# smithzvk/gsl-scattered-interpolation

Measured on AMD Instinct MI355X. Metric: M interpolated points/sec (whole hot path: fill + solve + eval sweep per step), higher is better.
Workload: dtype f64; 1 GPU; C3: 3-D N=16384 Gaussian RBF (16k x 16k fp64 Cholesky), M=1M targets per GPU; config=C3, n_centres=16384, dim=3, targets_per_gpu=1000000, targets_total=1000000, parallelism=1 GPU

## Files before the change

gsl-scattered-interpolation_amd/csrc/hip/chol.hip:

```cpp
#include "common.h"
#include <math.h>
#include <stdlib.h>

#ifdef SINTERP_DIAG_PROF
__device__ unsigned long long g_diag_ts[80];
#define TSTAMP(i) do { if (threadIdx.x == 0) g_diag_ts[i] = __builtin_readcyclecounter(); } while (0)
extern "C" int gsl_sinterp_hip_debug_diag_ts(unsigned long long *out) { return (int)hipMemcpyFromSymbol(out, HIP_SYMBOL(g_diag_ts), sizeof(unsigned long long) * 80); }
#endif
#include "chol_potrf.h"

#define TRSV_MAXR 5


__global__ void __launch_bounds__(256)
chol_base_kernel(double *__restrict__ A, size_t lda, size_t n, size_t j0, int nb, int *__restrict__ info,
                 double *__restrict__ diag_store)
{
  __shared__ double sL[CB][CB + 1];
  __shared__ double sInv[CB];
  const int tid = threadIdx.x;

  const size_t row = j0 + nb + (size_t)blockIdx.x * blockDim.x + tid;
  double *p = A + row * lda + j0;
  double x[CB];
  const bool vecrow = nb == CB && ((((uintptr_t)p) & 15) == 0) && ((lda & 1) == 0);
  if (row < n) {
    if (vecrow) {
#pragma unroll
      for (int k = 0; k < CB; k += 2) { const double2 t = *reinterpret_cast<const double2 *>(p + k); x[k] = t.x; x[k + 1] = t.y; }
    } else {
#pragma unroll
      for (int k = 0; k < CB; k++) x[k] = k < nb ? p[k] : 0.0;
    }
  }

  if (tid < 64) {
    const int lane = tid;
    double a[CB];
#pragma unroll
    for (int k = 0; k < CB; k++) a[k] = (lane < nb && k <= lane && k < nb) ? A[(j0 + lane) * lda + j0 + k] : 0.0;
    bool bad = false;
#pragma unroll
    for (int j = 0; j < CB; j++) {
      double v = a[j];
#pragma unroll
      for (int k = 0; k < j; k++) v = fma(-a[k], lane_bcast(a[k], j), v);
      double d = lane_bcast(v, j);
      if (j < nb && !(d > 0.0)) {
        if (lane == 0 && blockIdx.x == 0) atomicCAS(info, 0, (int)(j0 + j + 1));
        bad = true;
        d = 1.0;
      }
      if (j >= nb) d = 1.0;
      double y = __builtin_amdgcn_rsq(d);
      y = y * fma(-0.5 * d * y, y, 1.5);
      y = y * fma(-0.5 * d * y, y, 1.5);
      double sd = d * y;
      sd = fma(fma(-sd, sd, d), 0.5 * y, sd);
      const double inv = fma(fma(-sd, y, 1.0), y, y);
      a[j] = (lane == j) ? sd : v * inv;
      if (lane == 0) sInv[j] = inv;
    }
    (void)bad;
    if (lane < CB) {
#pragma unroll
      for (int k = 0; k < CB; k++) sL[lane][k] = (k <= lane) ? a[k] : 0.0;
      if (blockIdx.x == 0) {
        double *dst = diag_store + (j0 / CB) * (CB * CB) + lane * CB;
#pragma unroll
        for (int k = 0; k < CB; k++) dst[k] = (k <= lane) ? a[k] : 0.0;
      }
    }
  }
  __syncthreads();

  if (row >= n) return;
#pragma unroll
  for (int j = 0; j < CB; j++) {
    double v = x[j];
#pragma unroll
    for (int k = 0; k < j; k++) v = fma(-x[k], sL[j][k], v);
    x[j] = v * sInv[j];
  }
  if (vecrow) {
#pragma unroll
    for (int k = 0; k < CB; k += 2) *reinterpret_cast<double2 *>(p + k) = make_double2(x[k], x[k + 1]);
  } else {
#pragma unroll
    for (int k = 0; k < CB; k++) if (k < nb) p[k] = x[k];
  }
}

__global__ void __launch_bounds__(256)
chol_diag_writeback_kernel(double *__restrict__ A, size_t lda, size_t n, const double *__restrict__ diag_store)
{
  const size_t j0 = (size_t)blockIdx.x * CB;
  for (int e = threadIdx.x; e < CB * CB; e += 256) {
    const int r = e / CB, k = e % CB;
    if (k <= r && j0 + r < n) A[(j0 + r) * lda + j0 + k] = diag_store[(size_t)blockIdx.x * (CB * CB) + e];
  }
}


__device__ __forceinline__ void diag128_forward(const double *S, const double *Dv, double *fs, double *tt, int tid, int nrhs)
{
  const int lane = tid & 63, wave = tid >> 6, r = lane & 31, half = lane >> 5;
  for (int q = wave; q < nrhs; q += 4) {
    double *y = fs + q * PB, *t = tt + q * CB;
#pragma unroll
    for (int i = 0; i < 4; i++) {
      double sum = 0.0;
#pragma unroll
      for (int kb = 0; kb < i; kb++) {
        const double *Lr = S + pblk(i, kb) + r * PQ + half * 16;
        const double *yk = y + kb * 32 + half * 16;
#pragma unroll
        for (int k = 0; k < 16; k += 2) {
          const double2 l2 = *reinterpret_cast<const double2 *>(Lr + k);
          sum = fma(l2.x, yk[k], sum);
          sum = fma(l2.y, yk[k + 1], sum);
        }
      }
      sum += __shfl_xor(sum, 32);
      if (half == 0) t[r] = y[i * 32 + r] - sum;
      __builtin_amdgcn_wave_barrier();
      const double *Wr = Dv + i * PBLK + (half * 16) * PQ + r;
      double acc = 0.0;
#pragma unroll
      for (int c = 0; c < 16; c++) acc = fma(Wr[c * PQ], t[half * 16 + c], acc);
      acc += __shfl_xor(acc, 32);
      if (half == 0) y[i * 32 + r] = acc;
      __builtin_amdgcn_wave_barrier();
    }
  }
}

__global__ void __launch_bounds__(256)
chol_diag128_kernel(double *__restrict__ A, size_t lda, size_t j0, int *__restrict__ info, double *__restrict__ diag_store,
                    double *__restrict__ Dinvg, double *__restrict__ fb, size_t ldf, int nrhs)
{
  extern __shared__ __attribute__((aligned(16))) double sm[];
  double *S = sm;
  double *Dv = S + 10 * PBLK;
  double *fs = Dv + 4 * PBLK;
  double *tt = fs + 5 * PB;
  const int tid = threadIdx.x;
  double *Ab = A + j0 * lda + j0;
  TSTAMP(0);

  {
    double v[40], fv[3];
    const int r8 = tid >> 5, k = tid & 31;
#pragma unroll
    for (int t = 0; t < 40; t++) {
      constexpr int BI[10] = {0, 1, 1, 2, 2, 2, 3, 3, 3, 3}, BJ[10] = {0, 0, 1, 0, 1, 2, 0, 1, 2, 3};
      const int b = t >> 2, r = (t & 3) * 8 + r8;
      v[t] = Ab[(size_t)(BI[b] * 32 + r) * lda + BJ[b] * 32 + k];
    }
#pragma unroll
    for (int t = 0; t < 3; t++) { const int e = t * 256 + tid; fv[t] = e < nrhs * PB ? fb[(size_t)(e >> 7) * ldf + j0 + (e & 127)] : 0.0; }
#pragma unroll
    for (int t = 0; t < 40; t++) S[(t >> 2) * PBLK + ((t & 3) * 8 + r8) * PQ + k] = v[t];
#pragma unroll
    for (int t = 0; t < 16; t++) { const int r = (t & 3) * 8 + r8; Dv[(t >> 2) * PBLK + r * PQ + k] = r == k ? 1.0 : 0.0; }
#pragma unroll
    for (int t = 0; t < 3; t++) { const int e = t * 256 + tid; if (e < nrhs * PB) fs[e] = fv[t]; }
  }
  __syncthreads();
  TSTAMP(1);

  potrf128_lds<4>(S, Dv, tid, info, j0);

  TSTAMP(18);
  if (nrhs > 0) {
    diag128_forward(S, Dv, fs, tt, tid, nrhs);
    __syncthreads();
  }
  {
    const int r8 = tid >> 5, k = tid & 31;
#pragma unroll
    for (int t = 0; t < 40; t++) {
      constexpr int BI[10] = {0, 1, 1, 2, 2, 2, 3, 3, 3, 3}, BJ[10] = {0, 0, 1, 0, 1, 2, 0, 1, 2, 3};
      const int b = t >> 2, r = (t & 3) * 8 + r8, bi = BI[b], bj = BJ[b];
      const double v = S[b * PBLK + r * PQ + k];
      if (bi != bj || k <= r) Ab[(size_t)(bi * 32 + r) * lda + bj * 32 + k] = v;
      if (bi == bj && diag_store) diag_store[(j0 / CB + bi) * (CB * CB) + r * CB + k] = (k <= r) ? v : 0.0;
    }
#pragma unroll
    for (int t = 0; t < 16; t++) {
      const int b = t >> 2, r = (t & 3) * 8 + r8;
      Dinvg[b * 1024 + r * 32 + k] = Dv[b * PBLK + k * PQ + r];
    }
#pragma unroll
    for (int t = 0; t < 3; t++) { const int e = t * 256 + tid; if (e < nrhs * PB) fb[(size_t)(e >> 7) * ldf + j0 + (e & 127)] = fs[e]; }
  }
  TSTAMP(19);
}

#define TRX 130
#define TRY 34
template <int RF>
__global__ void __launch_bounds__(256)
chol_trsm16_kernel(double *__restrict__ A, size_t lda, size_t n, size_t j0, const double *__restrict__ Dinvg, size_t row_start,
                   double *__restrict__ fb, size_t ldf, int nrhs)
{
  constexpr bool KSPLIT = RF == 1;
  constexpr int NP = KSPLIT ? 2 : 1;
  constexpr int NRF = KSPLIT ? 1 : RF / 2;
  constexpr int ROWS = 16 * RF;
  constexpr int LCH = KSPLIT ? 4 : 8;
  extern __shared__ __attribute__((aligned(16))) double sm[];
  double *Xp = sm;
  double *Yp = Xp + NP * ROWS * TRX;
  double *ys = Yp + NP * ROWS * TRY;
  const int tid = threadIdx.x, lane = tid & 63, wave = tid >> 6;
  const int f = wave & 1, g = wave >> 1, fr = lane & 15, fq = lane >> 4;
  const int plane = KSPLIT ? g : 0;
  const size_t row0 = row_start + (size_t)blockIdx.x * ROWS;
  const int dch = KSPLIT ? (f ? 4 : 2) : (f ? 8 : 4);
  const int dk0 = KSPLIT ? dch * g : 0, lk0 = KSPLIT ? 4 * g : 0;

  double a0[NRF][8], dv[4][8], lb[6][LCH], yv[3];
  double4_t cinit[NRF][3];
#pragma unroll
  for (int c = 0; c < 4; c++)
#pragma unroll
    for (int i = 0; i < 8; i++) dv[c][i] = i < dch ? Dinvg[c * 1024 + (16 * f + fr) * 32 + 4 * (dk0 + i) + fq] : 0.0;
#pragma unroll
  for (int c = 1; c < 4; c++)
#pragma unroll
    for (int p = 0; p < c; p++)
#pragma unroll
      for (int i = 0; i < LCH; i++)
        lb[c * (c - 1) / 2 + p][i] = A[(j0 + 32 * c + 16 * f + fr) * lda + j0 + 32 * p + 4 * (lk0 + i) + fq];
#pragma unroll
  for (int t = 0; t < NRF; t++) {
    const int rf = KSPLIT ? 0 : g + 2 * t;
    const size_t arow = row0 + 16 * rf + fr < n ? row0 + 16 * rf + fr : n - 1;
    const double *Arow = A + arow * lda + j0;
#pragma unroll
    for (int i = 0; i < 8; i++) a0[t][i] = i < dch ? Arow[4 * (dk0 + i) + fq] : 0.0;
#pragma unroll
    for (int c = 1; c < 4; c++)
#pragma unroll
      for (int rg = 0; rg < 4; rg++) {
        const size_t r = row0 + 16 * rf + fq + 4 * rg < n ? row0 + 16 * rf + fq + 4 * rg : n - 1;
        cinit[t][c - 1][rg] = plane == 0 ? A[r * lda + j0 + 32 * c + 16 * f + fr] : 0.0;
      }
  }
#pragma unroll
  for (int t = 0; t < 3; t++) { const int e = t * 256 + tid; yv[t] = e < nrhs * PB ? fb[(size_t)(e >> 7) * ldf + j0 + (e & 127)] : 0.0; }
#pragma unroll
  for (int t = 0; t < 3; t++) { const int e = t * 256 + tid; if (e < nrhs * PB) ys[e] = yv[t]; }

  double facc[RF][TRSV_MAXR];
#pragma unroll
  for (int t = 0; t < RF; t++)
#pragma unroll
    for (int q = 0; q < TRSV_MAXR; q++) facc[t][q] = 0.0;
  const int sr = tid >> 4, sc = (tid & 15) * 2;

#pragma unroll
  for (int c = 0; c < 4; c++) {
    if (c > 0) {
#pragma unroll
      for (int t = 0; t < NRF; t++) {
        const int rf = KSPLIT ? 0 : g + 2 * t;
        double4_t acc = cinit[t][c - 1];
#pragma unroll
        for (int p = 0; p < c; p++)
#pragma unroll
          for (int i = 0; i < LCH; i++) {
            const int k = 32 * p + 4 * (lk0 + i) + fq;
            double a = Xp[(16 * rf + fr) * TRX + k];
            if constexpr (KSPLIT) a += Xp[ROWS * TRX + (16 * rf + fr) * TRX + k];
            acc = __builtin_amdgcn_mfma_f64_16x16x4f64(-a, lb[c * (c - 1) / 2 + p][i], acc, 0, 0, 0);
          }
#pragma unroll
        for (int rg = 0; rg < 4; rg++) Yp[plane * ROWS * TRY + (16 * rf + fq + 4 * rg) * TRY + 16 * f + fr] = acc[rg];
      }
      __syncthreads();
    }
#pragma unroll
    for (int t = 0; t < NRF; t++) {
      const int rf = KSPLIT ? 0 : g + 2 * t;
      double4_t x = (double4_t){0.0, 0.0, 0.0, 0.0};
#pragma unroll
      for (int i = 0; i < 8; i++) {
        if (i < dch) {
          const int k = 4 * (dk0 + i) + fq;
          double a = a0[t][i];
          if (c > 0) {
            a = Yp[(16 * rf + fr) * TRY + k];
            if constexpr (KSPLIT) a += Yp[ROWS * TRY + (16 * rf + fr) * TRY + k];
          }
          x = __builtin_amdgcn_mfma_f64_16x16x4f64(a, dv[c][i], x, 0, 0, 0);
        }
      }
#pragma unroll
      for (int rg = 0; rg < 4; rg++) Xp[plane * ROWS * TRX + (16 * rf + fq + 4 * rg) * TRX + 32 * c + 16 * f + fr] = x[rg];
    }
    __syncthreads();
#pragma unroll
    for (int t = 0; t < RF; t++) {
      const int r = sr + 16 * t;
      double2 xv = *reinterpret_cast<const double2 *>(&Xp[r * TRX + 32 * c + sc]);
      if constexpr (KSPLIT) {
        const double2 x1 = *reinterpret_cast<const double2 *>(&Xp[ROWS * TRX + r * TRX + 32 * c + sc]);
        xv.x += x1.x; xv.y += x1.y;
      }
      const size_t grow = row0 + r;
      if (grow < n) *reinterpret_cast<double2 *>(A + grow * lda + j0 + 32 * c + sc) = xv;
#pragma unroll
      for (int q = 0; q < TRSV_MAXR; q++)
        if (q < nrhs) facc[t][q] = fma(xv.y, ys[q * PB + 32 * c + sc + 1], fma(xv.x, ys[q * PB + 32 * c + sc], facc[t][q]));
    }
  }
  if (nrhs > 0) {
#pragma unroll
    for (int t = 0; t < RF; t++) {
      const size_t grow = row0 + sr + 16 * t;
#pragma unroll
      for (int q = 0; q < TRSV_MAXR; q++) {
        if (q < nrhs) {
          double v = facc[t][q];
          v += __shfl_xor(v, 1);
          v += __shfl_xor(v, 2);
          v += __shfl_xor(v, 4);
          v += __shfl_xor(v, 8);
          if ((tid & 15) == 0 && grow < n) fb[(size_t)q * ldf + grow] -= v;
        }
      }
    }
  }
}

template <int RF>
static int launch_trsm16(gsl_sinterp_hip_ctx *ctx, double *A, size_t lda, size_t n, size_t j0, const double *d_linv, size_t row_start,
                         double *fb, size_t ldf, int nrhs)
{
  constexpr int NP = RF == 1 ? 2 : 1;
  const size_t lds = (size_t)(NP * 16 * RF * (TRX + TRY) + TRSV_MAXR * PB) * sizeof(double);
  { int ast = sinterp_func_lds(ctx, (const void *)chol_trsm16_kernel<RF>, (int)lds); if (ast) return ast; }
  const size_t below = n - row_start;
  hipLaunchKernelGGL(chol_trsm16_kernel<RF>, dim3((unsigned)((below + 16 * RF - 1) / (16 * RF))), dim3(256), lds, ctx->stream, A, lda, n, j0,
                     d_linv, row_start, fb, ldf, nrhs);
  return ST_SUCCESS;
}

__global__ void __launch_bounds__(256)
chol_trsm128_kernel(double *__restrict__ A, size_t lda, size_t n, size_t j0, const double *__restrict__ Dinvg, size_t row_start,
                    double *__restrict__ fb, size_t ldf, int nrhs)
{
  extern __shared__ __attribute__((aligned(16))) double sm[];
  double *Bt = sm;
  double *Lb = Bt + 64 * TR_LD;
  double *Dvb = Lb + 6 * PBLK;
  double *ys = Dvb + 4 * PBLK;
  const int tid = threadIdx.x, lane = tid & 63, wave = tid >> 6;
  const int fr = lane & 15, fq = lane >> 4;
  const size_t row0 = row_start + (size_t)blockIdx.x * 64;
  {
    double2 vb[16];
    double vl[24], vd[16], yv[3];
    const int r8 = tid >> 5, k = tid & 31;
#pragma unroll
    for (int t = 0; t < 16; t++) {
      const int e = t * 256 + tid, r = e >> 6, k2 = (e & 63) * 2;
      const size_t grow = row0 + r < n ? row0 + r : n - 1;
      vb[t] = *reinterpret_cast<const double2 *>(A + grow * lda + j0 + k2);
    }
#pragma unroll
    for (int t = 0; t < 24; t++) {
      constexpr int BI[6] = {1, 2, 2, 3, 3, 3}, BJ[6] = {0, 0, 1, 0, 1, 2};
      const int b = t >> 2, r = (t & 3) * 8 + r8;
      vl[t] = A[(j0 + BI[b] * 32 + r) * lda + j0 + BJ[b] * 32 + k];
    }
#pragma unroll
    for (int t = 0; t < 16; t++) vd[t] = Dinvg[(t >> 2) * 1024 + ((t & 3) * 8 + r8) * 32 + k];
#pragma unroll
    for (int t = 0; t < 3; t++) { const int e = t * 256 + tid; yv[t] = e < nrhs * PB ? fb[(size_t)(e >> 7) * ldf + j0 + (e & 127)] : 0.0; }
#pragma unroll
    for (int t = 0; t < 16; t++) {
      const int e = t * 256 + tid, r = e >> 6, k2 = (e & 63) * 2;
      Bt[r * TR_LD + k2] = vb[t].x; Bt[r * TR_LD + k2 + 1] = vb[t].y;
    }
#pragma unroll
    for (int t = 0; t < 3; t++) { const int e = t * 256 + tid; if (e < nrhs * PB) ys[e] = yv[t]; }
#pragma unroll
    for (int t = 0; t < 24; t++) Lb[(t >> 2) * PBLK + ((t & 3) * 8 + r8) * PQ + k] = vl[t];
#pragma unroll
    for (int t = 0; t < 16; t++) Dvb[(t >> 2) * PBLK + ((t & 3) * 8 + r8) * PQ + k] = vd[t];
  }
  __syncthreads();

  double *arow = Bt + (wave * 16 + fr) * TR_LD + fq;
  double *drow = Bt + (wave * 16 + fq) * TR_LD + fr;
#pragma unroll
  for (int c = 0; c < 4; c++) {
    double4_t acc[2];
#pragma unroll
    for (int f = 0; f < 2; f++)
#pragma unroll
      for (int rg = 0; rg < 4; rg++) acc[f][rg] = drow[4 * rg * TR_LD + c * 32 + f * 16];
#pragma unroll
    for (int p = 0; p < c; p++) {
      const double *lb = Lb + (c * (c - 1) / 2 + p) * PBLK + fr * PQ + fq;
#pragma unroll
      for (int kk = 0; kk < 8; kk++) {
        const double a = -arow[p * 32 + kk * 4];
#pragma unroll
        for (int f = 0; f < 2; f++) acc[f] = __builtin_amdgcn_mfma_f64_16x16x4f64(a, lb[f * 16 * PQ + kk * 4], acc[f], 0, 0, 0);
      }
    }
#pragma unroll
    for (int f = 0; f < 2; f++)
#pragma unroll
      for (int rg = 0; rg < 4; rg++) drow[4 * rg * TR_LD + c * 32 + f * 16] = acc[f][rg];
    const double *db = Dvb + c * PBLK + fr * PQ + fq;
#pragma unroll
    for (int f = 0; f < 2; f++) {
      acc[f] = (double4_t){0.0, 0.0, 0.0, 0.0};
#pragma unroll
      for (int kk = 0; kk < (f + 1) * 4; kk++)
        acc[f] = __builtin_amdgcn_mfma_f64_16x16x4f64(arow[c * 32 + kk * 4], db[f * 16 * PQ + kk * 4], acc[f], 0, 0, 0);
    }
#pragma unroll
    for (int f = 0; f < 2; f++)
#pragma unroll
      for (int rg = 0; rg < 4; rg++) {
        drow[4 * rg * TR_LD + c * 32 + f * 16] = acc[f][rg];
        const size_t grow = row0 + wave * 16 + fq + 4 * rg;
        if (grow < n) A[grow * lda + j0 + c * 32 + f * 16 + fr] = acc[f][rg];
      }
  }
  if (nrhs > 0) {
    __syncthreads();
    const int r = tid >> 2, qd = tid & 3;
    const size_t grow = row0 + r;
    for (int q = 0; q < nrhs; q++) {
      double v = 0.0;
#pragma unroll
      for (int k = 0; k < 32; k++) v = fma(Bt[r * TR_LD + qd * 32 + k], ys[q * PB + qd * 32 + k], v);
      v += __shfl_xor(v, 1);
      v += __shfl_xor(v, 2);
      if (qd == 0 && grow < n) fb[(size_t)q * ldf + grow] -= v;
    }
  }
}


__global__ void __launch_bounds__(256)
tricpy_lower_to_upper_kernel(double *__restrict__ A, size_t lda, size_t n)
{
  __shared__ double tile[32][33];
  const size_t bi = blockIdx.y, bj = blockIdx.x;
  if (bj > bi) return;
  const int tx = threadIdx.x & 31, ty = threadIdx.x >> 5;
  for (int r = ty; r < 32; r += 8) {
    const size_t i = bi * 32 + r, j = bj * 32 + tx;
    tile[r][tx] = (i < n && j < n) ? A[i * lda + j] : 0.0;
  }
  __syncthreads();
  for (int r = ty; r < 32; r += 8) {
    const size_t j = bj * 32 + r, i = bi * 32 + tx;
    if (i < n && j < n && j < i) A[j * lda + i] = tile[tx][r];
  }
}

static size_t chol_split(size_t w)
{
  const size_t unit = w > PB ? PB : CB;
  size_t w1 = ((w / 2 + unit - 1) / unit) * unit;
  if (w1 >= w) w1 = w - unit;
  return w1;
}

static int chol_panel(gsl_sinterp_hip_ctx *ctx, double *A, size_t lda, size_t n, size_t j0, size_t w, int *d_info,
                      double *d_diag, double *fb, size_t ldf, int nrhs)
{
  int st;
  static const bool no_p128 = getenv("GSL_SINTERP_NO_PANEL128") && getenv("GSL_SINTERP_NO_PANEL128")[0] == '1';
  if (w == PB && !no_p128 && (lda & 1) == 0 && ((((uintptr_t)(A + j0 * lda + j0)) & 15) == 0)) {
    double *d_linv = d_diag + ((n + CB - 1) / CB) * (CB * CB);
    const size_t lds_diag = (size_t)(14 * PBLK + TRSV_MAXR * (PB + CB)) * sizeof(double);
    { int ast = sinterp_func_lds(ctx, (const void *)chol_diag128_kernel, (int)lds_diag); if (ast) return ast; }
    hipLaunchKernelGGL(chol_diag128_kernel, dim3(1), dim3(256), lds_diag, ctx->stream, A, lda, j0, d_info,
                       n % PB == 0 ? (double *)NULL : d_diag, d_linv, fb, ldf, nrhs);
    const size_t below = n - j0 - w;
    if (below) {
      static const int force_rf = getenv("GSL_SINTERP_TRSM_RF") ? atoi(getenv("GSL_SINTERP_TRSM_RF")) : 0;
      int ast = 0;
      if (force_rf == 1 || (!force_rf && below <= 4096)) ast = launch_trsm16<1>(ctx, A, lda, n, j0, d_linv, j0 + PB, fb, ldf, nrhs);
      else if (force_rf == 2) ast = launch_trsm16<2>(ctx, A, lda, n, j0, d_linv, j0 + PB, fb, ldf, nrhs);
      else if (force_rf == 4) ast = launch_trsm16<4>(ctx, A, lda, n, j0, d_linv, j0 + PB, fb, ldf, nrhs);
      else {
        const size_t lds_trsm = (size_t)(64 * TR_LD + 10 * PBLK + TRSV_MAXR * PB) * sizeof(double);
        ast = sinterp_func_lds(ctx, (const void *)chol_trsm128_kernel, (int)lds_trsm);
        if (!ast)
          hipLaunchKernelGGL(chol_trsm128_kernel, dim3((unsigned)((below + 63) / 64)), dim3(256), lds_trsm, ctx->stream, A, lda, n, j0,
                             (const double *)d_linv, j0 + PB, fb, ldf, nrhs);
      }
      if (ast) return ast;
    }
    LAUNCH_CHECK(ctx);
    return ST_SUCCESS;
  }
  if (w <= PB) {
    if (fb) return sinterp_fail(ctx, ST_EFAILED, "cholesky: folded forward substitution on a panel that is not 128 wide", hipSuccess, __FILE__, __LINE__);
  }
  if (w <= CB) {
    const size_t below = n - j0 - w;
    const unsigned grid = (unsigned)((below + 255) / 256) + (below == 0 ? 1u : 0u);
    hipLaunchKernelGGL(chol_base_kernel, dim3(grid ? grid : 1), dim3(256), 0, ctx->stream, A, lda, n, j0, (int)w, d_info, d_diag);
    LAUNCH_CHECK(ctx);
    return ST_SUCCESS;
  }
  const size_t w1 = chol_split(w);
  st = chol_panel(ctx, A, lda, n, j0, w1, d_info, d_diag, fb, ldf, nrhs);
  if (st) return st;
  const size_t r0 = j0 + w1, w2 = w - w1;
  st = sinterp_gemm_minus(ctx, n - r0, w2, w1, A + r0 * lda + j0, lda, A + r0 * lda + j0, lda, 0, A + r0 * lda + r0, lda, 1);
  if (st) return st;
  return chol_panel(ctx, A, lda, n, r0, w2, d_info, d_diag, fb, ldf, nrhs);
}

static bool chol_fold_applicable(size_t n, const double *d_a, size_t lda, int nrhs)
{
  static const bool no_p128 = getenv("GSL_SINTERP_NO_PANEL128") && getenv("GSL_SINTERP_NO_PANEL128")[0] == '1';
  static const bool no_fold = getenv("GSL_SINTERP_NO_FOLD") && getenv("GSL_SINTERP_NO_FOLD")[0] == '1';
  return !no_p128 && !no_fold && nrhs >= 1 && nrhs <= TRSV_MAXR && n >= PB && n % PB == 0 && (lda & 1) == 0 && ((((uintptr_t)d_a) & 15) == 0);
}


__global__ void chol_zero_info_kernel(int *info) { *info = 0; }

static int chol_read_info(gsl_sinterp_hip_ctx *ctx, size_t n, int *h_info)
{
  int *d_info = (int *)ctx->d_scratch + 8;
  int info = 0;
  HIP_OK(ctx, hipStreamSynchronize(ctx->stream));
  HIP_OK(ctx, hipMemcpy(&info, d_info, sizeof(int), hipMemcpyDeviceToHost));
  HIP_OK(ctx, hipStreamSynchronize(ctx->stream));
  if (h_info) *h_info = info;
  if (info) {
    snprintf(ctx->err, sizeof ctx->err, "cholesky_decomp1: matrix is not positive definite (pivot %d of %zu <= 0)", info, n);
    return ST_EDOM;
  }
  return ST_SUCCESS;
}

static int cholesky_decomp1_impl(gsl_sinterp_hip_ctx *ctx, size_t n, double *d_a, size_t lda, int *h_info, bool symmetric_input,
                                 double *fb, size_t ldf, int nrhs, int *h_folded, bool defer_info = false)
{
  if (h_folded) *h_folded = 0;
  REQUIRE(ctx, ctx != NULL, ST_EFAULT);
  HIP_OK(ctx, hipSetDevice(ctx->device));
  EXCLUSIVE_SECTION(ctx);
  REQUIRE(ctx, lda >= n, ST_EINVAL);
  REQUIRE(ctx, n == 0 || d_a, ST_EFAULT);
  if (h_info) *h_info = 0;
  if (n == 0) return ST_SUCCESS;
  int *d_info = (int *)ctx->d_scratch + 8;
  const size_t nblk = (n + CB - 1) / CB;
  void *d_diag = NULL;
  const size_t n_pan = (n + PB - 1) / PB;
  int st = sinterp_workspace(ctx, (nblk * CB * CB + (n_pan + 1) * (4 * 1024)) * sizeof(double), &d_diag);
  if (st) return st;
  st = sinterp_streamk_prepare(ctx);
  if (st) return st;
  const bool fold = fb != NULL && chol_fold_applicable(n, d_a, lda, nrhs) && ldf >= n;
  if (!fold) { fb = NULL; ldf = 0; nrhs = 0; }
  int replayed = 0;
  const sinterp_graph_key gkey = {{n, lda, (uintptr_t)d_a, (uintptr_t)fb, ldf, (uintptr_t)nrhs, (uintptr_t)(symmetric_input ? 1 : 0)}};
  st = sinterp_graph_try_launch(ctx, 0, gkey, &replayed);
  if (st) return st;
  if (!replayed) {
    hipStream_t saved;
    st = sinterp_capture_begin(ctx, &saved);
    if (st) return st;
    hipLaunchKernelGGL(chol_zero_info_kernel, dim3(1), dim3(1), 0, ctx->stream, d_info);
    hipError_t me = hipSuccess;
    const unsigned nt = (unsigned)((n + 31) / 32);
    if (!symmetric_input) hipLaunchKernelGGL(tricpy_lower_to_upper_kernel, dim3(nt, nt), dim3(256), 0, ctx->stream, d_a, lda, n);
    st = chol_panel(ctx, d_a, lda, n, 0, n, d_info, (double *)d_diag, fb, ldf, nrhs);
    {
      static const bool no_p128w = getenv("GSL_SINTERP_NO_PANEL128") && getenv("GSL_SINTERP_NO_PANEL128")[0] == '1';
      const bool all128 = !no_p128w && n % PB == 0 && (lda & 1) == 0 && ((((uintptr_t)d_a) & 15) == 0);
      if (!all128)
        hipLaunchKernelGGL(chol_diag_writeback_kernel, dim3((unsigned)nblk), dim3(256), 0, ctx->stream, d_a, lda, n,
                           (const double *)d_diag);
    }
    int st2 = sinterp_capture_end(ctx, saved, 0, gkey);
    if (me != hipSuccess) return sinterp_fail(ctx, ST_EFAILED, "zero info", me, __FILE__, __LINE__);
    if (st) return st;
    if (st2) return st2;
    LAUNCH_CHECK(ctx);
  }
  if (h_folded) *h_folded = fold ? 1 : 0;
  if (defer_info) return ST_SUCCESS;
  st = chol_read_info(ctx, n, h_info);
  if (st && h_folded) *h_folded = 0;
  return st;
}

extern "C" int gsl_sinterp_hip_cholesky_decomp1(gsl_sinterp_hip_ctx *ctx, size_t n, double *d_a, size_t lda, int *h_info)
{
  return cholesky_decomp1_impl(ctx, n, d_a, lda, h_info, false, NULL, 0, 0, NULL);
}

int sinterp_cholesky_decomp1_sym(gsl_sinterp_hip_ctx *ctx, size_t n, double *d_a, size_t lda, int *h_info)
{
  return cholesky_decomp1_impl(ctx, n, d_a, lda, h_info, true, NULL, 0, 0, NULL);
}

static int chol_factor_solve(gsl_sinterp_hip_ctx *ctx, size_t n, double *d_a, size_t lda, int *h_info, double *d_x, size_t ldx,
                             int nrhs, bool symmetric_input)
{
  EXCLUSIVE_SECTION(ctx);
  int folded = 0;
  int st = cholesky_decomp1_impl(ctx, n, d_a, lda, h_info, symmetric_input, d_x, ldx, nrhs, &folded, true);
  if (st) return st;
  if (!folded) st = sinterp_cholesky_svx_multi(ctx, n, d_a, lda, d_x, ldx, nrhs);
  else st = sinterp_trsv_multi(ctx, n, d_a, lda, d_x, d_x, ldx, nrhs, 1, 0);
  if (st) return st;
  return chol_read_info(ctx, n, h_info);
}

int sinterp_cholesky_factor_solve_sym(gsl_sinterp_hip_ctx *ctx, size_t n, double *d_a, size_t lda, int *h_info, double *d_x, size_t ldx,
                                      int nrhs)
{
  return chol_factor_solve(ctx, n, d_a, lda, h_info, d_x, ldx, nrhs, true);
}

extern "C" int gsl_sinterp_hip_cholesky_factor_solve(gsl_sinterp_hip_ctx *ctx, size_t n, double *d_a, size_t lda, int *h_info,
                                                     double *d_x, size_t ldx, int nrhs)
{
  REQUIRE(ctx, ctx != NULL, ST_EFAULT);
  HIP_OK(ctx, hipSetDevice(ctx->device));
  REQUIRE(ctx, lda >= n && ldx >= n && nrhs >= 1 && nrhs <= TRSV_MAXR, ST_EINVAL);
  REQUIRE(ctx, n == 0 || (d_a && d_x), ST_EFAULT);
  if (h_info) *h_info = 0;
  if (n == 0) return ST_SUCCESS;
  return chol_factor_solve(ctx, n, d_a, lda, h_info, d_x, ldx, nrhs, false);
}

#define TS 64

__global__ void __launch_bounds__(256)
trsv_sweep_kernel(const double *__restrict__ T, size_t ldt, size_t n, double *__restrict__ b,
                  double *__restrict__ xout, size_t ldb, int nrhs, size_t j0, int nb, int mode, int unit)
{
  __shared__ double sx[TRSV_MAXR][TS];
  __shared__ double sD[TS][TS + 1];
  const int tid = threadIdx.x;
  for (int e = tid; e < TS * TS; e += 256) {
    const int r = e / TS, c = e % TS;
    double v = 0.0;
    if (r < nb && c < nb) v = T[(j0 + r) * ldt + j0 + c];
    sD[r][c] = v;
  }
  __syncthreads();
  {
    const int lane = tid & 63, wave = tid >> 6;
    const double dl = (lane < nb && !unit) ? sD[lane][lane] : 1.0;
    const double rl = 1.0 / dl;
    for (int r = wave; r < nrhs; r += 4) {
      double bi = lane < nb ? b[r * ldb + j0 + lane] : 0.0;
#define TRSV_STEP(J, COEF, COND)                                   \
      {                                                            \
        const double bj = lane_bcast(bi, (J));                     \
        double xj = bj;                                            \
        if (!unit) {                                               \
          const double dj = lane_bcast(dl, (J)), rj = lane_bcast(rl, (J)); \
          const double q = bj * rj;                                \
          xj = fma(fma(-dj, q, bj), rj, q);                        \
        }                                                          \
        if (lane == (J)) bi = xj;                                  \
        if (COND) bi = fma(-(COEF), xj, bi);                       \
      }
      if (mode == 0) {
        for (int j = 0; j < nb; j++) TRSV_STEP(j, sD[lane][j], lane > j)
      } else if (mode == 1) {
        for (int j = nb - 1; j >= 0; j--) TRSV_STEP(j, sD[j][lane], lane < j)
      } else {
        for (int j = nb - 1; j >= 0; j--) TRSV_STEP(j, sD[lane][j], lane < j)
      }
#undef TRSV_STEP
      if (lane < nb) { sx[r][lane] = bi; if (blockIdx.x == 0) xout[r * ldb + j0 + lane] = bi; }
    }
  }
  __syncthreads();

  if (mode == 1) {
    __shared__ double s_part[TRSV_MAXR][4][64];
    const int il = tid & 63, jg = tid >> 6;
    const size_t i = (size_t)blockIdx.x * 64 + il;
    double acc[TRSV_MAXR];
#pragma unroll
    for (int r = 0; r < TRSV_MAXR; r++) acc[r] = 0.0;
    if (i < j0) {
      const int jb = jg * 16;
      double t[16];
#pragma unroll
      for (int jj = 0; jj < 16; jj++)
        t[jj] = (jb + jj < nb) ? T[(j0 + jb + jj) * ldt + i] : 0.0;
#pragma unroll
      for (int jj = 0; jj < 16; jj++)
#pragma unroll
        for (int r = 0; r < TRSV_MAXR; r++) if (r < nrhs) acc[r] = fma(t[jj], sx[r][jb + jj], acc[r]);
    }
#pragma unroll
    for (int r = 0; r < TRSV_MAXR; r++) if (r < nrhs) s_part[r][jg][il] = acc[r];
    __syncthreads();
    if (jg == 0 && i < j0) {
#pragma unroll
      for (int r = 0; r < TRSV_MAXR; r++)
        if (r < nrhs) b[r * ldb + i] -= (s_part[r][0][il] + s_part[r][1][il]) + (s_part[r][2][il] + s_part[r][3][il]);
    }
  } else {
    const int lane = tid & 63, wave = tid >> 6;
    const int rsub = lane >> 3, c8 = (lane & 7) * 8;
    const size_t base = (mode == 0) ? j0 + nb : 0;
    const size_t limit = (mode == 0) ? n : j0;
#pragma unroll
    for (int pass = 0; pass < 2; pass++) {
      const size_t i = base + ((size_t)blockIdx.x * 2 + pass) * 32 + wave * 8 + rsub;
      double acc[TRSV_MAXR];
#pragma unroll
      for (int r = 0; r < TRSV_MAXR; r++) acc[r] = 0.0;
      if (i < limit) {
        const double *row = T + i * ldt + j0 + c8;
        double t[8];
        if (nb == TS && ((((uintptr_t)row) & 15) == 0)) {
#pragma unroll
          for (int k = 0; k < 8; k += 2) { const double2 v = *reinterpret_cast<const double2 *>(row + k); t[k] = v.x; t[k + 1] = v.y; }
        } else {
#pragma unroll
          for (int k = 0; k < 8; k++) t[k] = (c8 + k < nb) ? row[k] : 0.0;
        }
#pragma unroll
        for (int r = 0; r < TRSV_MAXR; r++)
          if (r < nrhs) {
#pragma unroll
            for (int k = 0; k < 8; k++) acc[r] = fma(t[k], sx[r][c8 + k], acc[r]);
          }
      }
#pragma unroll
      for (int r = 0; r < TRSV_MAXR; r++) {
        if (r < nrhs) {
          double a = acc[r];
          a += __shfl_xor(a, 1);
          a += __shfl_xor(a, 2);
          a += __shfl_xor(a, 4);
          if (i < limit && (lane & 7) == 0) b[r * ldb + i] -= a;
        }
      }
    }
  }
}

__global__ void __launch_bounds__(64)
tri_inv_kernel(const double *__restrict__ T, size_t ldt, size_t n, int upper, int unit, double *__restrict__ Dinv)
{
  __shared__ double sL[TS][TS + 1];
  const size_t j0 = (size_t)blockIdx.x * TS;
  const int nb = (int)((n - j0) < TS ? (n - j0) : TS);
  const int lane = threadIdx.x;
  {
    double tv[TS];
    const int lc = lane < nb ? lane : nb - 1;
#pragma unroll
    for (int r = 0; r < TS; r++) {
      const int rc = r < nb ? r : nb - 1;
      tv[r] = upper ? T[(j0 + lc) * ldt + j0 + rc] : T[(j0 + rc) * ldt + j0 + lc];
    }
#pragma unroll
    for (int r = 0; r < TS; r++) {
      double v = (r == lane) ? 1.0 : 0.0;
      if (r < nb && lane < nb) v = lane < r ? tv[r] : (lane == r ? (unit ? 1.0 : tv[r]) : 0.0);
      sL[r][lane] = v;
    }
  }
  __syncthreads();
  double x[TS];
#pragma unroll
  for (int i = 0; i < TS; i++) {
    double v = (i == lane) ? 1.0 : 0.0;
#pragma unroll
    for (int k = 0; k < i; k++) v = fma(-sL[i][k], x[k], v);
    x[i] = v / sL[i][i];
  }
  double *out = Dinv + (size_t)blockIdx.x * TS * TS;
#pragma unroll
  for (int i = 0; i < TS; i++) out[(size_t)i * TS + lane] = x[i];
}

__global__ void __launch_bounds__(256)
trsv_sweep_inv_kernel(const double *__restrict__ T, size_t ldt, size_t n, double *__restrict__ b,
                      double *__restrict__ xout, size_t ldb, int nrhs, size_t j0, int nb, int mode,
                      const double *__restrict__ Dinv)
{
  __shared__ double sx[TRSV_MAXR][TS];
  __shared__ double sb[TRSV_MAXR][TS];
  __shared__ double sW[TS][TS + 1];
  const int tid = threadIdx.x, lane = tid & 63, wave = tid >> 6;

  double t[16];
  size_t irow = 0;
  bool have = false;
  const int rsub = lane >> 3, c8 = (lane & 7) * 8;
  if (mode == 1) {
    irow = (size_t)blockIdx.x * 64 + lane;
    have = irow < j0;
#pragma unroll
    for (int jj = 0; jj < 16; jj++)
      t[jj] = (have && wave * 16 + jj < nb) ? T[(j0 + wave * 16 + jj) * ldt + irow] : 0.0;
  } else {
    const size_t base = (mode == 0) ? j0 + nb : 0;
    const size_t limit = (mode == 0) ? n : j0;
#pragma unroll
    for (int pass = 0; pass < 2; pass++) {
      const size_t i = base + ((size_t)blockIdx.x * 2 + pass) * 32 + wave * 8 + rsub;
      const double *row = T + i * ldt + j0 + c8;
#pragma unroll
      for (int k = 0; k < 8; k++) t[pass * 8 + k] = (i < limit && c8 + k < nb) ? row[k] : 0.0;
    }
  }
  const double *D = Dinv + (j0 / TS) * (size_t)(TS * TS);
  for (int e = tid; e < TS * TS; e += 256) {
    const int r = e / TS, c = e % TS;
    sW[r][c] = D[e];
  }
  for (int e = tid; e < nrhs * TS; e += 256) {
    const int r = e / TS, c = e % TS;
    sb[r][c] = c < nb ? b[r * ldb + j0 + c] : 0.0;
  }
  __syncthreads();
  for (int r = wave; r < nrhs; r += 4) {
    double acc = 0.0;
    if (mode == 0) { for (int c = 0; c < TS; c++) acc = fma(sW[lane][c], sb[r][c], acc); }
    else { for (int c = 0; c < TS; c++) acc = fma(sW[c][lane], sb[r][c], acc); }
    sx[r][lane] = acc;
    if (blockIdx.x == 0 && lane < nb) xout[r * ldb + j0 + lane] = acc;
  }
  __syncthreads();
  if (mode == 1) {
    __shared__ double s_part[TRSV_MAXR][4][64];
#pragma unroll
    for (int r = 0; r < TRSV_MAXR; r++) {
      if (r < nrhs) {
        double acc = 0.0;
#pragma unroll
        for (int jj = 0; jj < 16; jj++) acc = fma(t[jj], sx[r][wave * 16 + jj], acc);
        s_part[r][wave][lane] = acc;
      }
    }
    __syncthreads();
    if (wave == 0 && have) {
#pragma unroll
      for (int r = 0; r < TRSV_MAXR; r++)
        if (r < nrhs) b[r * ldb + irow] -= (s_part[r][0][lane] + s_part[r][1][lane]) + (s_part[r][2][lane] + s_part[r][3][lane]);
    }
  } else {
    const size_t base = (mode == 0) ? j0 + nb : 0;
    const size_t limit = (mode == 0) ? n : j0;
#pragma unroll
    for (int pass = 0; pass < 2; pass++) {
      const size_t i = base + ((size_t)blockIdx.x * 2 + pass) * 32 + wave * 8 + rsub;
#pragma unroll
      for (int r = 0; r < TRSV_MAXR; r++) {
        if (r < nrhs) {
          double a = 0.0;
#pragma unroll
          for (int k = 0; k < 8; k++) a = fma(t[pass * 8 + k], sx[r][c8 + k], a);
          a += __shfl_xor(a, 1);
          a += __shfl_xor(a, 2);
          a += __shfl_xor(a, 4);
          if (i < limit && (lane & 7) == 0) b[r * ldb + i] -= a;
        }
      }
    }
  }
}

__global__ void __launch_bounds__(256)
trsv_dataflow_kernel(const double *__restrict__ T, size_t ldt, size_t n, const double *__restrict__ b, double *xout, size_t ldb,
                     int nrhs, int mode, const double *__restrict__ Dinv, unsigned *tf, unsigned long long *xq, unsigned nblk)
{
  const unsigned want = __hip_atomic_load(tf, __ATOMIC_RELAXED, __HIP_MEMORY_SCOPE_AGENT) + 1u;
  const size_t npad = (size_t)nblk * TS;
  __shared__ double sx[2][TRSV_MAXR][TS];
  __shared__ double sW[TS][TS + 1];
  __shared__ double srhs[TRSV_MAXR][TS];
  __shared__ double s_part[TRSV_MAXR][4][TS];
  const int tid = threadIdx.x, lane = tid & 63, wave = tid >> 6;
  const int rsub = lane >> 3, c8 = (lane & 7) * 8;
  for (unsigned t = blockIdx.x; t < nblk; t += gridDim.x) {
    const unsigned I = (mode == 0) ? t : nblk - 1 - t;
    const size_t i0 = (size_t)I * TS;
    const int nbI = (int)((n - i0) < TS ? (n - i0) : TS);
    __syncthreads();
    for (int e = tid; e < TS * TS; e += 256) sW[e / TS][e % TS] = Dinv[(size_t)I * (TS * TS) + e];
    double bpre[(TRSV_MAXR * TS + 255) / 256];
#pragma unroll
    for (int q = 0; q < (TRSV_MAXR * TS + 255) / 256; q++) {
      const int e = q * 256 + tid, r = e / TS, c = e % TS;
      bpre[q] = (e < nrhs * TS && c < nbI) ? b[r * ldb + i0 + c] : 0.0;
    }
    double acc[TRSV_MAXR][2];
#pragma unroll
    for (int r = 0; r < TRSV_MAXR; r++) acc[r][0] = acc[r][1] = 0.0;
    for (unsigned sstep = 0; sstep < t; sstep++) {
      const unsigned J = (mode == 0) ? sstep : nblk - 1 - sstep;
      const size_t j0 = (size_t)J * TS;
      double tt[16];
      if (mode == 1) {
#pragma unroll
        for (int jj = 0; jj < 16; jj++) {
          const size_t jr = j0 + wave * 16 + jj;
          tt[jj] = (jr < n && lane < nbI) ? T[jr * ldt + i0 + lane] : 0.0;
        }
      } else {
#pragma unroll
        for (int pass = 0; pass < 2; pass++) {
          const size_t i = i0 + pass * 32 + wave * 8 + rsub;
          const double *row = T + i * ldt + j0 + c8;
          if (i < n && j0 + TS <= n && ((((uintptr_t)row) & 15) == 0)) {
#pragma unroll
            for (int k = 0; k < 8; k += 2) { const double2 v = *reinterpret_cast<const double2 *>(row + k); tt[pass * 8 + k] = v.x; tt[pass * 8 + k + 1] = v.y; }
          } else {
#pragma unroll
            for (int k = 0; k < 8; k++) tt[pass * 8 + k] = (i < n && j0 + c8 + k < n) ? row[k] : 0.0;
          }
        }
      }
      const int buf = sstep & 1;
      for (int e = tid; e < nrhs * TS; e += 256) {
        const int r = e / TS, c = e % TS;
        double v = 0.0;
        if (j0 + c < n) {
          const unsigned long long *q = xq + 2 * ((size_t)r * npad + j0 + c);
          unsigned long long w0, w1;
          for (;;) {
            w0 = __hip_atomic_load(q, __ATOMIC_RELAXED, __HIP_MEMORY_SCOPE_AGENT);
            w1 = __hip_atomic_load(q + 1, __ATOMIC_RELAXED, __HIP_MEMORY_SCOPE_AGENT);
            if ((unsigned)(w0 >> 32) == want && (unsigned)(w1 >> 32) == want) break;
            __builtin_amdgcn_s_sleep(1);
          }
          v = __hiloint2double((int)(unsigned)w1, (int)(unsigned)w0);
        }
        sx[buf][r][c] = v;
      }
      __syncthreads();
      if (mode == 1) {
#pragma unroll
        for (int r = 0; r < TRSV_MAXR; r++)
          if (r < nrhs) {
#pragma unroll
            for (int jj = 0; jj < 16; jj++) acc[r][0] = fma(tt[jj], sx[buf][r][wave * 16 + jj], acc[r][0]);
          }
      } else {
#pragma unroll
        for (int r = 0; r < TRSV_MAXR; r++)
          if (r < nrhs) {
#pragma unroll
            for (int pass = 0; pass < 2; pass++)
#pragma unroll
              for (int k = 0; k < 8; k++) acc[r][pass] = fma(tt[pass * 8 + k], sx[buf][r][c8 + k], acc[r][pass]);
          }
      }
    }
    if (mode == 1) {
#pragma unroll
      for (int r = 0; r < TRSV_MAXR; r++) if (r < nrhs) s_part[r][wave][lane] = acc[r][0];
      __syncthreads();
#pragma unroll
      for (int q = 0; q < (TRSV_MAXR * TS + 255) / 256; q++) {
        const int e = q * 256 + tid, r = e / TS, c = e % TS;
        if (e < nrhs * TS) {
          const double sum = (s_part[r][0][c] + s_part[r][1][c]) + (s_part[r][2][c] + s_part[r][3][c]);
          srhs[r][c] = (c < nbI) ? bpre[q] - sum : 0.0;
        }
      }
    } else {
#pragma unroll
      for (int r = 0; r < TRSV_MAXR; r++)
        if (r < nrhs) {
#pragma unroll
          for (int pass = 0; pass < 2; pass++) {
            double a = acc[r][pass];
            a += __shfl_xor(a, 1);
            a += __shfl_xor(a, 2);
            a += __shfl_xor(a, 4);
            const int row = pass * 32 + wave * 8 + rsub;
            if ((lane & 7) == 0) srhs[r][row] = -a;
          }
        }
      __syncthreads();
#pragma unroll
      for (int q = 0; q < (TRSV_MAXR * TS + 255) / 256; q++) {
        const int e = q * 256 + tid, r = e / TS, c = e % TS;
        if (e < nrhs * TS) srhs[r][c] = (c < nbI) ? bpre[q] + srhs[r][c] : 0.0;
      }
    }
    __syncthreads();
    for (int r = wave; r < nrhs; r += 4) {
      double p0 = 0.0, p1 = 0.0, p2 = 0.0, p3 = 0.0;
      if (mode == 0) {
#pragma unroll
        for (int c = 0; c < TS; c += 4) {
          p0 = fma(sW[lane][c], srhs[r][c], p0); p1 = fma(sW[lane][c + 1], srhs[r][c + 1], p1);
          p2 = fma(sW[lane][c + 2], srhs[r][c + 2], p2); p3 = fma(sW[lane][c + 3], srhs[r][c + 3], p3);
        }
      } else {
#pragma unroll
        for (int c = 0; c < TS; c += 4) {
          p0 = fma(sW[c][lane], srhs[r][c], p0); p1 = fma(sW[c + 1][lane], srhs[r][c + 1], p1);
          p2 = fma(sW[c + 2][lane], srhs[r][c + 2], p2); p3 = fma(sW[c + 3][lane], srhs[r][c + 3], p3);
        }
      }
      if (lane < nbI) {
        const double xv = (p0 + p1) + (p2 + p3);
        unsigned long long *q = xq + 2 * ((size_t)r * npad + i0 + lane);
        const unsigned long long tag = (unsigned long long)want << 32;
        __hip_atomic_store(q, tag | (unsigned)__double2loint(xv), __ATOMIC_RELAXED, __HIP_MEMORY_SCOPE_AGENT);
        __hip_atomic_store(q + 1, tag | (unsigned)__double2hiint(xv), __ATOMIC_RELAXED, __HIP_MEMORY_SCOPE_AGENT);
        xout[r * ldb + i0 + lane] = xv;
      }
    }
    if (t == nblk - 1) {
      __syncthreads();
      if (tid == 0) __hip_atomic_store(tf, want, __ATOMIC_RELAXED, __HIP_MEMORY_SCOPE_AGENT);
    }
  }
}

static int trsv_launches(gsl_sinterp_hip_ctx *ctx, size_t n, const double *T, size_t ldt, double *b, double *xout,
                         size_t ldb, int nrhs, int mode, int unit, double *d_inv, int inv_ready)
{
  const size_t nblk = (n + TS - 1) / TS;
  const bool use_inv = nblk > 1 && d_inv != NULL;
  if (use_inv && !inv_ready) {
    hipLaunchKernelGGL(tri_inv_kernel, dim3((unsigned)nblk), dim3(64), 0, ctx->stream, T, ldt, n, mode == 2 ? 1 : 0, unit, d_inv);
    LAUNCH_CHECK(ctx);
  }
  static const bool no_df = getenv("GSL_SINTERP_NO_DATAFLOW_TRSV") && getenv("GSL_SINTERP_NO_DATAFLOW_TRSV")[0] == '1';
  if (use_inv && !no_df && ctx->sk_wgs > 0 && ctx->d_tf && ctx->tf_count >= nblk + 1 && ctx->d_xq) {
    const unsigned G = (unsigned)(nblk < (size_t)ctx->sk_wgs ? nblk : (size_t)ctx->sk_wgs);
    hipLaunchKernelGGL(trsv_dataflow_kernel, dim3(G), dim3(256), 0, ctx->stream, T, ldt, n, (const double *)b, xout, ldb, nrhs, mode,
                       (const double *)d_inv, ctx->d_tf, ctx->d_xq, (unsigned)nblk);
    LAUNCH_CHECK(ctx);
    return ST_SUCCESS;
  }
  for (size_t t = 0; t < nblk; t++) {
    const size_t blk = (mode == 0) ? t : nblk - 1 - t;
    const size_t j0 = blk * TS;
    const int nb = (int)((n - j0) < TS ? (n - j0) : TS);
    const size_t rest = (mode == 0) ? n - j0 - nb : j0;
    const unsigned grid = (unsigned)((rest + 63) / 64);
    if (use_inv)
      hipLaunchKernelGGL(trsv_sweep_inv_kernel, dim3(grid ? grid : 1), dim3(256), 0, ctx->stream, T, ldt, n, b, xout, ldb, nrhs,
                         j0, nb, mode, (const double *)d_inv);
    else
      hipLaunchKernelGGL(trsv_sweep_kernel, dim3(grid ? grid : 1), dim3(256), 0, ctx->stream, T, ldt, n, b, xout, ldb, nrhs, j0,
                         nb, mode, unit);
    LAUNCH_CHECK(ctx);
  }
  return ST_SUCCESS;
}

__global__ void __launch_bounds__(256)
vec_copy_kernel(const double *__restrict__ src, double *__restrict__ dst, size_t count)
{
  const size_t i = (size_t)blockIdx.x * 256 + threadIdx.x;
  if (i < count) dst[i] = src[i];
}

static int trsv_multi_ex(gsl_sinterp_hip_ctx *ctx, size_t n, const double *T, size_t ldt, double *b, double *xout, size_t ldb,
                         int nrhs, int mode, int unit, int inv_ready)
{
  if (n == 0 || nrhs == 0) return ST_SUCCESS;
  if (nrhs > TRSV_MAXR) return sinterp_fail(ctx, ST_EINVAL, "trsv: too many right-hand sides", hipSuccess, __FILE__, __LINE__);
  const int slot = mode == 0 ? 2 : 3;
  const sinterp_graph_key gkey = {{n, ldt, (uintptr_t)T, (uintptr_t)b, (uintptr_t)xout, ldb, (uintptr_t)nrhs, (uintptr_t)mode,
                                    (uintptr_t)unit, (uintptr_t)inv_ready}};
  int replayed = 0;
  int st = sinterp_graph_try_launch(ctx, slot, gkey, &replayed);
  if (st || replayed) return st;
  void *d_inv = NULL;
  const size_t inv_bytes = ((n + TS - 1) / TS) * TS * TS * sizeof(double);
  const bool in_place = b == xout;
  if (in_place && inv_ready) return sinterp_fail(ctx, ST_EINVAL, "trsv: in-place sweep cannot reuse inverted blocks", hipSuccess, __FILE__, __LINE__);
  st = sinterp_invbuf(ctx, inv_bytes + (in_place ? (size_t)nrhs * ldb * sizeof(double) : 0), &d_inv);
  if (st) return st;
  {
    const size_t need = (n + TS - 1) / TS + 1;
    if (need > ctx->tf_count) {
      HIP_OK(ctx, hipStreamSynchronize(ctx->stream));
      if (ctx->d_tf) { HIP_OK(ctx, hipFree(ctx->d_tf)); ctx->d_tf = NULL; ctx->tf_count = 0; }
      const size_t cnt = need < 1024 ? 1024 : need * 2;
      HIP_OK(ctx, hipMalloc((void **)&ctx->d_tf, cnt * sizeof(unsigned)));
      HIP_OK(ctx, hipMemset(ctx->d_tf, 0, cnt * sizeof(unsigned)));
      if (ctx->d_xq) { HIP_OK(ctx, hipFree(ctx->d_xq)); ctx->d_xq = NULL; }
      const size_t xq_bytes = (size_t)TRSV_MAXR * cnt * TS * 2 * sizeof(unsigned long long);
      HIP_OK(ctx, hipMalloc((void **)&ctx->d_xq, xq_bytes));
      HIP_OK(ctx, hipMemset(ctx->d_xq, 0, xq_bytes));
      HIP_OK(ctx, hipDeviceSynchronize());
      ctx->tf_count = cnt;
      for (int i = 2; i < 4; i++)
        if (ctx->graph[i].exec) { (void)hipGraphExecDestroy(ctx->graph[i].exec); ctx->graph[i].exec = NULL; }
    }
  }
  st = sinterp_streamk_prepare(ctx);
  if (st) return st;
  double *b_src = in_place ? (double *)((char *)d_inv + inv_bytes) : b;
  hipStream_t saved;
  st = sinterp_capture_begin(ctx, &saved);
  if (st) return st;
  if (in_place) {
    const size_t cnt = (size_t)(nrhs - 1) * ldb + n;
    hipLaunchKernelGGL(vec_copy_kernel, dim3((unsigned)((cnt + 255) / 256)), dim3(256), 0, ctx->stream, (const double *)b, b_src, cnt);
  }
  st = trsv_launches(ctx, n, T, ldt, b_src, xout, ldb, nrhs, mode, unit, (double *)d_inv, inv_ready);
  int st2 = sinterp_capture_end(ctx, saved, slot, gkey);
  return st ? st : st2;
}

int sinterp_trsv_multi(gsl_sinterp_hip_ctx *ctx, size_t n, const double *T, size_t ldt, double *b, double *xout, size_t ldb,
                       int nrhs, int mode, int unit)
{
  return trsv_multi_ex(ctx, n, T, ldt, b, xout, ldb, nrhs, mode, unit, 0);
}

int sinterp_trsv(gsl_sinterp_hip_ctx *ctx, size_t n, const double *T, size_t ldt, double *b, double *xout, int mode,
                 int unit)
{
  return sinterp_trsv_multi(ctx, n, T, ldt, b, xout, n, 1, mode, unit);
}

int sinterp_cholesky_svx_multi(gsl_sinterp_hip_ctx *ctx, size_t n, const double *d_llt, size_t lda, double *d_x, size_t ldx,
                               int nrhs)
{
  EXCLUSIVE_SECTION(ctx);
  void *d_tmp = NULL;
  int st = sinterp_workspace(ctx, (size_t)nrhs * ldx * sizeof(double), &d_tmp);
  if (st) return st;
  st = sinterp_trsv_multi(ctx, n, d_llt, lda, d_x, (double *)d_tmp, ldx, nrhs, 0, 0);
  if (st) return st;
  return trsv_multi_ex(ctx, n, d_llt, lda, (double *)d_tmp, d_x, ldx, nrhs, 1, 0, 1);
}

extern "C" int gsl_sinterp_hip_cholesky_svx(gsl_sinterp_hip_ctx *ctx, size_t n, const double *d_llt, size_t lda, double *d_x)
{
  REQUIRE(ctx, ctx != NULL, ST_EFAULT);
  HIP_OK(ctx, hipSetDevice(ctx->device));
  EXCLUSIVE_SECTION(ctx);
  REQUIRE(ctx, lda >= n, ST_EINVAL);
  REQUIRE(ctx, n == 0 || (d_llt && d_x), ST_EFAULT);
  return sinterp_cholesky_svx_multi(ctx, n, d_llt, lda, d_x, n, 1);
}
```

gsl-scattered-interpolation_amd/csrc/hip/chol_potrf.h:

```cpp
#ifndef SINTERP_CHOL_POTRF_H
#define SINTERP_CHOL_POTRF_H

#define CB 32
#ifndef TSTAMP
#define TSTAMP(i) do { } while (0)
#endif
#if defined(SINTERP_DIAG_PROF_COLS)
#define TSTAMP_COL(i) TSTAMP(i)
#else
#define TSTAMP_COL(i) do { } while (0)
#endif

__device__ __forceinline__ double lane_bcast(double v, int src)
{
  int lo = __builtin_amdgcn_readlane(__double2loint(v), src);
  int hi = __builtin_amdgcn_readlane(__double2hiint(v), src);
  return __hiloint2double(hi, lo);
}

typedef double double4_t __attribute__((ext_vector_type(4)));
#define PB 128
#define PQ 34
#define PBLK (32 * PQ)
#define TR_LD 130

__device__ __forceinline__ int pblk(int bi, int bj) { return (bi * (bi + 1) / 2 + bj) * PBLK; }

__device__ __forceinline__ double4_t frag_nt(const double *Ab, const double *Bb, int fi, int fj, int lane, double4_t acc, double sgn)
{
  const double *ap = Ab + (fi * 16 + (lane & 15)) * PQ + (lane >> 4);
  const double *bp = Bb + (fj * 16 + (lane & 15)) * PQ + (lane >> 4);
#pragma unroll
  for (int kk = 0; kk < 8; kk++) acc = __builtin_amdgcn_mfma_f64_16x16x4f64(sgn * ap[kk * 4], bp[kk * 4], acc, 0, 0, 0);
  return acc;
}
__device__ __forceinline__ double4_t frag_load(const double *Cb, int fi, int fj, int lane)
{
  double4_t c;
#pragma unroll
  for (int rg = 0; rg < 4; rg++) c[rg] = Cb[(fi * 16 + (lane >> 4) + 4 * rg) * PQ + fj * 16 + (lane & 15)];
  return c;
}
__device__ __forceinline__ void frag_store(double *Cb, int fi, int fj, int lane, double4_t c)
{
#pragma unroll
  for (int rg = 0; rg < 4; rg++) Cb[(fi * 16 + (lane >> 4) + 4 * rg) * PQ + fj * 16 + (lane & 15)] = c[rg];
}


#define PIN_V2(x, y)       asm volatile("" : "+v"(x), "+v"(y) : : "memory")
#define PIN_V4(x, y, z, w) asm volatile("" : "+v"(x), "+v"(y), "+v"(z), "+v"(w) : : "memory")
#define PIN_SSV(x, y, z)   asm volatile("" : "+s"(x), "+s"(y), "+v"(z) : : "memory")
#define PIN_SV(x, y)       asm volatile("" : "+s"(x), "+v"(y) : : "memory")

#define HB 16
template <int K0, int J>
__device__ __forceinline__ void potrf32_step(double (&a)[CB], double vprev, double cur, double inv_prev, double e, double e2, double q,
                                             const double *D, double *colp, const double (&rp)[CB])
{
  constexpr int END = K0 + HB;
  if constexpr (J < END) {
    TSTAMP_COL(32 + J);
    double v, d, uL2 = 0.0, acol = 0.0;
    if constexpr (J == K0) {
      v = cur;
      d = lane_bcast(v, J);
    } else {
      const double uL = e * inv_prev;
      d = fma(-uL, uL, q);
      acol = vprev * inv_prev;
      v = fma(-acol, uL, cur);
      uL2 = e2 * inv_prev;
    }
    double y0 = __builtin_amdgcn_rsq(d);
    PIN_V4(y0, v, uL2, acol);
    if constexpr (J > K0) { a[J - 1] = acol; colp[J - 1] = acol; }
    double rn[CB];
    if constexpr (J + 2 < END) {
#pragma unroll
      for (int k = K0; k < J; k += 2) {
        const double2 t2 = *reinterpret_cast<const double2 *>(D + (J + 2) * PQ + k);
        rn[k] = t2.x;
        if (k + 1 < CB) rn[k + 1] = t2.y;
      }
    }
    double en = 0.0, e2n = 0.0, qn = 0.0, curn = 0.0;
    if constexpr (J + 1 < END) en = lane_bcast(v, J + 1);
    if constexpr (J + 2 < END) e2n = lane_bcast(v, J + 2);
    if constexpr (J + 1 < END) {
      double p0 = a[J + 1], p1 = 0.0;
      if constexpr (J >= K0 + 1) p1 = -acol * uL2;
      PIN_SSV(en, e2n, p0);
#pragma unroll
      for (int k = K0; k + 1 < J; k++) {
        if (k & 1) p1 = fma(-a[k], rp[k], p1);
        else p0 = fma(-a[k], rp[k], p0);
      }
      curn = (J >= K0 + 1) ? p0 + p1 : p0;
      qn = lane_bcast(curn, J + 1);
      PIN_SV(qn, y0);
    }
    const double t = d * y0;
    const double rr = fma(-t, y0, 1.0);
    const double s1 = fma(0.375, rr, 0.5), u = y0 * rr;
    const double inv = fma(u, s1, y0);
    potrf32_step<K0, J + 1>(a, v, curn, inv, en, e2n, qn, D, colp, rn);
  } else {
    a[END - 1] = vprev * inv_prev;
    colp[END - 1] = a[END - 1];
  }
}

__device__ __forceinline__ void potrf32_split(double *D, double *Dt, int lane)
{
  const int fr = lane & 15, fq = lane >> 4;
  const double *ap = D + (HB + fr) * PQ + fq;
  const double *bp = Dt + fr * PQ + fq;
  double4_t cu, cw = (double4_t){0.0, 0.0, 0.0, 0.0};
#pragma unroll
  for (int rg = 0; rg < 4; rg++) cu[rg] = D[(HB + fq + 4 * rg) * PQ + HB + fr];
#pragma unroll
  for (int kk = 0; kk < 4; kk++) {
    const double av = ap[kk * 4], na = -av;
    cu = __builtin_amdgcn_mfma_f64_16x16x4f64(na, av, cu, 0, 0, 0);
    cw = __builtin_amdgcn_mfma_f64_16x16x4f64(na, bp[kk * 4], cw, 0, 0, 0);
  }
#pragma unroll
  for (int rg = 0; rg < 4; rg++) {
    D[(HB + fq + 4 * rg) * PQ + HB + fr] = cu[rg];
    Dt[fr * PQ + HB + fq + 4 * rg] = cw[rg];
  }
}


template <int NW>
__device__ __forceinline__ void potrf128_lds(double *S, double *Dv, int tid, int *__restrict__ info, size_t j0)
{
  const int lane = tid & 63, wave = tid >> 6;
  auto potrf_block = [&](int jb) {
    double *D = S + pblk(jb, jb);
    const bool is_row = lane < CB;
    double *Dt = Dv + jb * PBLK;
    double *colp = is_row ? D + lane * PQ : Dt + (lane - CB) * PQ;
    double a[CB];
#pragma unroll
    for (int k = 0; k < CB; k += 2) { const double2 t = *reinterpret_cast<const double2 *>(colp + k); a[k] = t.x; a[k + 1] = t.y; }
    double r0[CB];
    potrf32_step<0, 0>(a, 0.0, a[0], 0.0, 0.0, 0.0, 0.0, D, colp, r0);
    potrf32_split(D, Dt, lane);
#pragma unroll
    for (int k = HB; k < CB; k += 2) { const double2 t = *reinterpret_cast<const double2 *>(colp + k); a[k] = t.x; a[k + 1] = t.y; }
    potrf32_step<HB, HB>(a, 0.0, a[HB], 0.0, 0.0, 0.0, 0.0, D, colp, r0);
    const double dg = D[(lane & (CB - 1)) * PQ + (lane & (CB - 1))];
    const unsigned long long badm = __ballot(is_row && !(dg > 0.0));
    if (badm && lane == 0) atomicCAS(info, 0, (int)(j0 + jb * 32 + __ffsll((long long)badm)));
  };
  auto update_frag = [&](int jb, int bi, int bj, int f) {
    double *Cb = S + pblk(bi, bj);
    double4_t c = frag_load(Cb, f >> 1, f & 1, lane);
    c = frag_nt(S + pblk(bi, jb), S + pblk(bj, jb), f >> 1, f & 1, lane, c, -1.0);
    frag_store(Cb, f >> 1, f & 1, lane, c);
  };

  for (int jb = -1; jb < 3; jb++) {
    if (jb >= 0) {
    for (int u = wave; u < (3 - jb) * 2; u += NW) {
      double *Bb = S + pblk(jb + 1 + (u >> 1), jb);
      const int fi = u & 1;
      const double *ap = Bb + (fi * 16 + (lane & 15)) * PQ + (lane >> 4);
      const double *bp = Dv + jb * PBLK + (lane >> 4) * PQ + (lane & 15);
      double4_t x0 = (double4_t){0.0, 0.0, 0.0, 0.0}, x1 = x0;
#pragma unroll
      for (int kk = 0; kk < 8; kk++) {
        const double av = ap[kk * 4];
        if (kk < 4) x0 = __builtin_amdgcn_mfma_f64_16x16x4f64(av, bp[kk * 4 * PQ], x0, 0, 0, 0);
        x1 = __builtin_amdgcn_mfma_f64_16x16x4f64(av, bp[kk * 4 * PQ + 16], x1, 0, 0, 0);
      }
      frag_store(Bb, fi, 0, lane, x0);
      frag_store(Bb, fi, 1, lane, x1);
    }
    __syncthreads();
    TSTAMP(4 + jb * 4);
    if (wave < 3) update_frag(jb, jb + 1, jb + 1, wave == 0 ? 0 : wave + 1);
    __syncthreads();
    TSTAMP(5 + jb * 4);
    }
    if (wave == 0) {
      potrf_block(jb + 1);
    } else if (jb >= 0) {
      int unit = 0;
      for (int bi = jb + 2; bi < 4; bi++)
        for (int bj = jb + 1; bj <= bi; bj++)
          for (int f = 0; f < 4; f++) {
            if (bi == bj && f == 1) continue;
            if (unit++ % (NW - 1) == wave - 1) update_frag(jb, bi, bj, f);
          }
    }
    __syncthreads();
    TSTAMP(6 + jb * 4);
  }

}

#endif
```

gsl-scattered-interpolation_amd/csrc/hip/common.h:

```cpp
#ifndef SINTERP_HIP_COMMON_H
#define SINTERP_HIP_COMMON_H

#include <hip/hip_runtime.h>
#include <stdio.h>
#include <string.h>
#include "gsl_sinterp_hip.h"

enum { ST_SUCCESS = 0, ST_FAILURE = -1, ST_EDOM = 1, ST_EFAULT = 3, ST_EINVAL = 4, ST_EFAILED = 5, ST_ENOMEM = 8,
       ST_EBADLEN = 19 };

struct gsl_sinterp_hip_ctx {
  int device;
  hipStream_t stream;
  int owns_stream;
  hipEvent_t ev0, ev1;
  void *d_scratch;
  size_t scratch_bytes;
  void *d_work;
  size_t work_bytes;
  void *d_aux;
  size_t aux_bytes;
  void *d_inv;
  size_t inv_bytes;
  void *d_sort;
  size_t sort_bytes;
  void *d_sort2;
  size_t sort2_bytes;
  void *d_cent;
  size_t cent_bytes;
  struct { unsigned long long id; const void *x, *w; size_t n, xtda; int dim, kind; } cent_key;
  void *d_walk;
  size_t walk_bytes;
  hipStream_t side_stream;
  hipEvent_t side_ev[4];
  hipStream_t cap_stream;
  enum { GRAPH_KEY_WORDS = 12 };
  struct GraphSlot { hipGraphExec_t exec; uintptr_t key[GRAPH_KEY_WORDS]; } graph[4];
  int use_graphs;
  double *d_sk_partial;
  unsigned *d_sk_flags;
  int sk_wgs;
  unsigned *d_tf;
  size_t tf_count;
  unsigned long long *d_xq;
  void *d_lu_coop;
  void *d_jumpt;
  size_t jumpt_bytes;
  void *d_lw_a;
  void *d_lw_lines;
  size_t lw_a_bytes, lw_lines_bytes;
  const void *lw_rec;
  int lw_nodes, lw_Gs, lw_last;
  double lw_c[2], lw_lo[2], lw_w[2];
  const void *jump_rec;
  int jump_nodes, jump_G;
  int excl_depth;
  char err[512];
};

struct sinterp_graph_key {
  uintptr_t w[gsl_sinterp_hip_ctx::GRAPH_KEY_WORDS - 1];
};
int sinterp_graph_try_launch(gsl_sinterp_hip_ctx *ctx, int which, const sinterp_graph_key &key, int *launched);
int sinterp_capture_begin(gsl_sinterp_hip_ctx *ctx, hipStream_t *saved);
int sinterp_capture_end(gsl_sinterp_hip_ctx *ctx, hipStream_t saved, int which, const sinterp_graph_key &key);

static inline int sinterp_fail(gsl_sinterp_hip_ctx *ctx, int status, const char *what, hipError_t e,
                               const char *file, int line)
{
  if (ctx)
    snprintf(ctx->err, sizeof ctx->err, "%s: %s (%s:%d)", what, e == hipSuccess ? "invalid argument" : hipGetErrorString(e),
             file, line);
  return status;
}

#define HIP_OK(ctx, call)                                                               \
  do {                                                                                  \
    hipError_t _e = (call);                                                             \
    if (_e != hipSuccess)                                                               \
      return sinterp_fail(ctx, _e == hipErrorOutOfMemory ? ST_ENOMEM : ST_EFAILED, #call, _e, __FILE__, __LINE__); \
  } while (0)

#define REQUIRE(ctx, cond, status)                                                      \
  do {                                                                                  \
    if (!(cond)) return sinterp_fail(ctx, status, "requirement failed: " #cond, hipSuccess, __FILE__, __LINE__); \
  } while (0)

#define LAUNCH_CHECK(ctx) HIP_OK(ctx, hipGetLastError())

int sinterp_func_lds(gsl_sinterp_hip_ctx *ctx, const void *func, int bytes);

int sinterp_exclusive_begin(gsl_sinterp_hip_ctx *ctx);
int sinterp_exclusive_end(gsl_sinterp_hip_ctx *ctx);

struct SinterpExclusive {
  gsl_sinterp_hip_ctx *ctx;
  int st;
  explicit SinterpExclusive(gsl_sinterp_hip_ctx *c) : ctx(c), st(sinterp_exclusive_begin(c)) {}
  ~SinterpExclusive() { if (st == ST_SUCCESS) (void)sinterp_exclusive_end(ctx); }
  SinterpExclusive(const SinterpExclusive &) = delete;
  SinterpExclusive &operator=(const SinterpExclusive &) = delete;
};
#define EXCLUSIVE_SECTION(ctx) SinterpExclusive _excl(ctx); if (_excl.st) return _excl.st

int sinterp_rbf_fill_ex(gsl_sinterp_hip_ctx *ctx, int kind, double eps, const double *d_x, size_t n, int dim, size_t xtda,
                        double *d_phi, size_t lda, int lower_only);
int sinterp_tps_fill_shifted(gsl_sinterp_hip_ctx *ctx, const double *d_x, size_t n, int dim, size_t xtda, double *d_phi, size_t lda,
                             const double *d_Pk, int k, double cmul, unsigned long long *d_norm);

int sinterp_workspace(gsl_sinterp_hip_ctx *ctx, size_t bytes, void **out);

int sinterp_gemm_minus(gsl_sinterp_hip_ctx *ctx, size_t m, size_t n, size_t k, const double *A, size_t lda,
                       const double *B, size_t ldb, int b_is_kn, double *C, size_t ldc, int lower_only);

int sinterp_streamk_prepare(gsl_sinterp_hip_ctx *ctx);

int sinterp_trsv(gsl_sinterp_hip_ctx *ctx, size_t n, const double *T, size_t ldt, double *b, double *xout, int mode,
                 int unit);
int sinterp_trsv_multi(gsl_sinterp_hip_ctx *ctx, size_t n, const double *T, size_t ldt, double *b, double *xout, size_t ldb,
                       int nrhs, int mode, int unit);
int sinterp_cholesky_svx_multi(gsl_sinterp_hip_ctx *ctx, size_t n, const double *d_llt, size_t lda, double *d_x, size_t ldx,
                               int nrhs);
int sinterp_cholesky_decomp1_sym(gsl_sinterp_hip_ctx *ctx, size_t n, double *d_a, size_t lda, int *h_info);
int sinterp_cholesky_factor_solve_sym(gsl_sinterp_hip_ctx *ctx, size_t n, double *d_a, size_t lda, int *h_info, double *d_x, size_t ldx,
                                      int nrhs);
int sinterp_aux(gsl_sinterp_hip_ctx *ctx, size_t bytes, void **out);
int sinterp_invbuf(gsl_sinterp_hip_ctx *ctx, size_t bytes, void **out);
int sinterp_sortbuf(gsl_sinterp_hip_ctx *ctx, size_t bytes, void **out);
int sinterp_sort_targets(gsl_sinterp_hip_ctx *ctx, const double *d_y, size_t m, size_t ytda, int dim, int per_cell,
                         int **d_perm_out);
struct sinterp_sorted {
  double *ys;
  double *vs;
  int *ls;
  unsigned *cellid, *slot, *offset;
  unsigned long long *box;
  bool two_level;
  unsigned *inv;
  double *res1;
  unsigned *fin;
  unsigned *tl_cnt; unsigned tl_nb, tl_nwg, tl_ch;
};
int sinterp_sort_reorder(gsl_sinterp_hip_ctx *ctx, const double *d_y, size_t m, size_t ytda, int dim, int per_cell,
                         sinterp_sorted *out, size_t m_cap, int slot, const unsigned long long *box_in);
bool sinterp_sort_reorder_is_two_level(size_t m);
int sinterp_unsort(gsl_sinterp_hip_ctx *ctx, const sinterp_sorted *s, size_t m, double *d_values, int *d_leaf);
int sinterp_unsort_packed(gsl_sinterp_hip_ctx *ctx, const sinterp_sorted *s, size_t m, double *d_values, int *d_leaf);

int sinterp_sort_centres(gsl_sinterp_hip_ctx *ctx, const double *d_x, size_t n, size_t xtda, int dim, int per_cell,
                         int **d_perm_out);
int sinterp_sortbuf2(gsl_sinterp_hip_ctx *ctx, size_t bytes, void **out);
void sinterp_scan_u32(gsl_sinterp_hip_ctx *ctx, unsigned *count, size_t n, unsigned *runsum);
int sinterp_walkbuf(gsl_sinterp_hip_ctx *ctx, size_t bytes, void **out);
int sinterp_bbox_keys(gsl_sinterp_hip_ctx *ctx, const double *d_p, size_t n, size_t tda, int dim, unsigned long long *d_box);
int sinterp_centbuf(gsl_sinterp_hip_ctx *ctx, size_t bytes, void **out);

#endif
```

gsl-scattered-interpolation_amd/csrc/hip/gemm.hip:

```cpp
#include "common.h"
#include <stdlib.h>
#include <string.h>

typedef double double4_t __attribute__((ext_vector_type(4)));

#define GT_BM 128
#define GT_BN 128
#define GT_BK 16
#define GT_LDA (GT_BK + 2)
#define GT_LDBN (GT_BN + 16)
#define GT_ASZ (GT_BM * GT_LDA)
#define GT_BSZ 2304

struct GemmArgs {
  size_t m, n, k;
  const double *A; size_t lda;
  const double *B; size_t ldb;
  double *C; size_t ldc;
  int lower_only;
  int tiles_m, tiles_n;
  unsigned n_active;
};

__device__ __forceinline__ double2 ld2(const double *p, bool ok0, bool ok1, bool vec)
{
  if (vec && ok1) return *reinterpret_cast<const double2 *>(p);
  double2 v;
  v.x = ok0 ? p[0] : 0.0;
  v.y = ok1 ? p[1] : 0.0;
  return v;
}

template <int B_IS_KN, bool FULL>
__global__ void __launch_bounds__(256, 2)
gemm_minus_kernel(GemmArgs g)
{
  __shared__ __attribute__((aligned(16))) double sA[2][GT_ASZ];
  __shared__ __attribute__((aligned(16))) double sB[2][GT_BSZ];

  const unsigned nwg = gridDim.x, bid = blockIdx.x;
  const unsigned q = nwg / 8, r = nwg % 8, xcd = bid % 8;
  const unsigned tile = (xcd < r ? xcd * (q + 1) : r * (q + 1) + (xcd - r) * q) + bid / 8;
  int tm, tn;
  if (!g.lower_only) {
    tm = (int)(tile / g.tiles_n); tn = (int)(tile % g.tiles_n);
  } else {
    const unsigned tri = (unsigned)g.tiles_n * (unsigned)(g.tiles_n + 1) / 2;
    if (tile < tri) {
      tm = (int)((sqrt(8.0 * (double)tile + 1.0) - 1.0) * 0.5);
      while ((unsigned)(tm + 1) * (unsigned)(tm + 2) / 2 <= tile) tm++;
      while ((unsigned)tm * (unsigned)(tm + 1) / 2 > tile) tm--;
      tn = (int)(tile - (unsigned)tm * (unsigned)(tm + 1) / 2);
    } else {
      const unsigned t2 = tile - tri;
      tm = g.tiles_n + (int)(t2 / g.tiles_n); tn = (int)(t2 % g.tiles_n);
    }
  }

  const size_t row0 = (size_t)tm * GT_BM, col0 = (size_t)tn * GT_BN;
  const int tid = threadIdx.x, lane = tid & 63, wave = tid >> 6;
  const int wr = wave >> 1, wc = wave & 1;
  const int fr = lane & 15, fq = lane >> 4;

  const bool vecA = ((g.lda & 1) == 0) && ((((uintptr_t)g.A) & 15) == 0);
  const bool vecB = ((g.ldb & 1) == 0) && ((((uintptr_t)g.B) & 15) == 0);

  double4_t acc[4][4];
#pragma unroll
  for (int i = 0; i < 4; i++)
#pragma unroll
    for (int j = 0; j < 4; j++) acc[i][j] = (double4_t){0.0, 0.0, 0.0, 0.0};

  double2 ra[4], rb[4];

  auto fetch = [&](size_t k0) {
#pragma unroll
    for (int i = 0; i < 4; i++) {
      const int c = tid + 256 * i;
      if (FULL) {
        { const int rr = c >> 3, kc = (c & 7) * 2;
          ra[i] = *reinterpret_cast<const double2 *>(g.A + (row0 + rr) * g.lda + k0 + kc); }
        if (B_IS_KN) { const int kk = c >> 6, nc = (c & 63) * 2;
          rb[i] = *reinterpret_cast<const double2 *>(g.B + (k0 + kk) * g.ldb + col0 + nc); }
        else { const int rr = c >> 3, kc = (c & 7) * 2;
          rb[i] = *reinterpret_cast<const double2 *>(g.B + (col0 + rr) * g.ldb + k0 + kc); }
        continue;
      }
      {
        const int rr = c >> 3, kc = (c & 7) * 2;
        const size_t grow = row0 + rr, gk = k0 + kc;
        const bool okr = grow < g.m;
        ra[i] = ld2(g.A + grow * g.lda + gk, okr && gk < g.k, okr && gk + 1 < g.k, vecA);
      }
      if (B_IS_KN) {
        const int kk = c >> 6, nc = (c & 63) * 2;
        const size_t gk = k0 + kk, gcol = col0 + nc;
        const bool okk = gk < g.k;
        rb[i] = ld2(g.B + gk * g.ldb + gcol, okk && gcol < g.n, okk && gcol + 1 < g.n, vecB);
      } else {
        const int rr = c >> 3, kc = (c & 7) * 2;
        const size_t gn = col0 + rr, gk = k0 + kc;
        const bool okn = gn < g.n;
        rb[i] = ld2(g.B + gn * g.ldb + gk, okn && gk < g.k, okn && gk + 1 < g.k, vecB);
      }
    }
  };
  auto stash = [&](int buf) {
#pragma unroll
    for (int i = 0; i < 4; i++) {
      const int c = tid + 256 * i;
      { const int rr = c >> 3, kc = (c & 7) * 2;
        *reinterpret_cast<double2 *>(&sA[buf][rr * GT_LDA + kc]) = ra[i]; }
      if (B_IS_KN) { const int kk = c >> 6, nc = (c & 63) * 2;
        *reinterpret_cast<double2 *>(&sB[buf][kk * GT_LDBN + nc]) = rb[i]; }
      else { const int rr = c >> 3, kc = (c & 7) * 2;
        *reinterpret_cast<double2 *>(&sB[buf][rr * GT_LDA + kc]) = rb[i]; }
    }
  };

  const size_t nsteps = (g.k + GT_BK - 1) / GT_BK;
  fetch(0);
  stash(0);
  __syncthreads();

  for (size_t s = 0; s < nsteps; s++) {
    const int buf = (int)(s & 1);
    if (s + 1 < nsteps) fetch((s + 1) * GT_BK);
    const double *a_base = &sA[buf][(wr * 64 + fr) * GT_LDA + fq];
    const double *b_base = B_IS_KN ? &sB[buf][fq * GT_LDBN + wc * 64 + fr] : &sB[buf][(wc * 64 + fr) * GT_LDA + fq];
#pragma unroll
    for (int kk = 0; kk < GT_BK / 4; kk++) {
      double af[4], bf[4];
#pragma unroll
      for (int i = 0; i < 4; i++) af[i] = a_base[i * 16 * GT_LDA + kk * 4];
#pragma unroll
      for (int j = 0; j < 4; j++) bf[j] = B_IS_KN ? b_base[kk * 4 * GT_LDBN + j * 16] : b_base[j * 16 * GT_LDA + kk * 4];
#pragma unroll
      for (int i = 0; i < 4; i++)
#pragma unroll
        for (int j = 0; j < 4; j++)
          acc[i][j] = __builtin_amdgcn_mfma_f64_16x16x4f64(af[i], bf[j], acc[i][j], 0, 0, 0);
    }
    if (s + 1 < nsteps) stash(buf ^ 1);
    __syncthreads();
  }

#pragma unroll
  for (int i = 0; i < 4; i++) {
#pragma unroll
    for (int j = 0; j < 4; j++) {
      const size_t gcol = col0 + wc * 64 + j * 16 + fr;
#pragma unroll
      for (int rg = 0; rg < 4; rg++) {
        const size_t grow = row0 + wr * 64 + i * 16 + fq + 4 * rg;
        if ((FULL || (grow < g.m && gcol < g.n)) && (!g.lower_only || gcol <= grow)) {
          double *p = g.C + grow * g.ldc + gcol;
          *p = *p - acc[i][j][rg];
        }
      }
    }
  }
}


#define DM_STAGES 3

__device__ __forceinline__ void dma16(const double *gsrc, double *ldst)
{
  __builtin_amdgcn_global_load_lds((const __attribute__((address_space(1))) void *)gsrc,
                                   (__attribute__((address_space(3))) void *)ldst, 16, 0, 0);
}

template <int WR>
__global__ void __launch_bounds__(128 * WR, 1)
gemm_minus_dma_nt_kernel(GemmArgs g)
{
  constexpr int BM = 64 * WR;
  constexpr int NW = 2 * WR;
  constexpr int A_TILE = BM * GT_BK, B_TILE = GT_BN * GT_BK;
  constexpr int A_CH = BM / 8 / NW, B_CH = (GT_BN / 8) / NW;
  extern __shared__ __attribute__((aligned(16))) double smem[];
  double *sA = smem;
  double *sB = smem + DM_STAGES * A_TILE;

  const unsigned nwg = gridDim.x, bid = blockIdx.x;
  const unsigned q = nwg / 8, r = nwg % 8, xcd = bid % 8;
  const unsigned tile = (xcd < r ? xcd * (q + 1) : r * (q + 1) + (xcd - r) * q) + bid / 8;
  int tm, tn;
  if (!g.lower_only) {
    tm = (int)(tile / g.tiles_n); tn = (int)(tile % g.tiles_n);
  } else {
    constexpr unsigned R = BM / GT_BN;
    const unsigned full_rows = (unsigned)g.tiles_n / R;
    const unsigned tri = R * full_rows * (full_rows + 1) / 2;
    if (tile < tri) {
      const double t = (double)tile / (double)R;
      tm = (int)((sqrt(8.0 * t + 1.0) - 1.0) * 0.5);
      while (R * (unsigned)(tm + 1) * (unsigned)(tm + 2) / 2 <= tile) tm++;
      while (R * (unsigned)tm * (unsigned)(tm + 1) / 2 > tile) tm--;
      tn = (int)(tile - R * (unsigned)tm * (unsigned)(tm + 1) / 2);
    } else {
      const unsigned t2 = tile - tri;
      tm = (int)full_rows + (int)(t2 / g.tiles_n); tn = (int)(t2 % g.tiles_n);
    }
  }
  const size_t row0 = (size_t)tm * BM, col0 = (size_t)tn * GT_BN;
  const int tid = threadIdx.x, lane = tid & 63, wave = tid >> 6;
  const int wr = wave >> 1, wc = wave & 1;
  const int fr = lane & 15, fq = lane >> 4;

  const double *srcA[A_CH], *srcB[B_CH];
#pragma unroll
  for (int i = 0; i < A_CH; i++) {
    const int rr = (wave * A_CH + i) * 8 + (lane >> 3);
    srcA[i] = g.A + (row0 + rr) * g.lda + (((lane & 7) ^ ((rr >> 1) & 7)) << 1);
  }
#pragma unroll
  for (int i = 0; i < B_CH; i++) {
    const int rr = (wave * B_CH + i) * 8 + (lane >> 3);
    srcB[i] = g.B + (col0 + rr) * g.ldb + (((lane & 7) ^ ((rr >> 1) & 7)) << 1);
  }
  auto issue = [&](int stage, size_t k0) {
#pragma unroll
    for (int i = 0; i < A_CH; i++) dma16(srcA[i] + k0, sA + stage * A_TILE + (wave * A_CH + i) * 128);
#pragma unroll
    for (int i = 0; i < B_CH; i++) dma16(srcB[i] + k0, sB + stage * B_TILE + (wave * B_CH + i) * 128);
  };

  const int sw = (fr >> 1) & 7;
  int koff[4];
#pragma unroll
  for (int kk = 0; kk < 4; kk++) koff[kk] = (((kk * 2 + (fq >> 1)) ^ sw) << 1) + (fq & 1);
  const int arow = (wr * 64 + fr) * GT_BK, brow = (wc * 64 + fr) * GT_BK;

  double4_t acc[4][4];
#pragma unroll
  for (int i = 0; i < 4; i++)
#pragma unroll
    for (int j = 0; j < 4; j++) acc[i][j] = (double4_t){0.0, 0.0, 0.0, 0.0};

  const size_t nsteps = g.k / GT_BK;
  issue(0, 0);
  if (nsteps > 1) issue(1, GT_BK);

  for (size_t s = 0; s < nsteps; s++) {
    if (s + 1 < nsteps) {
      if (A_CH + B_CH == 8) asm volatile("s_waitcnt vmcnt(8)" ::: "memory");
      else asm volatile("s_waitcnt vmcnt(6)" ::: "memory");
    } else asm volatile("s_waitcnt vmcnt(0)" ::: "memory");
    __builtin_amdgcn_s_barrier();
    __builtin_amdgcn_sched_barrier(0);
    if (s + 2 < nsteps) issue((int)((s + 2) % DM_STAGES), (s + 2) * GT_BK);
    const double *a_base = sA + (s % DM_STAGES) * A_TILE + arow;
    const double *b_base = sB + (s % DM_STAGES) * B_TILE + brow;
#pragma unroll
    for (int kk = 0; kk < 4; kk++) {
      double af[4], bf[4];
#pragma unroll
      for (int i = 0; i < 4; i++) af[i] = a_base[i * 16 * GT_BK + koff[kk]];
#pragma unroll
      for (int j = 0; j < 4; j++) bf[j] = b_base[j * 16 * GT_BK + koff[kk]];
#pragma unroll
      for (int i = 0; i < 4; i++)
#pragma unroll
        for (int j = 0; j < 4; j++)
          acc[i][j] = __builtin_amdgcn_mfma_f64_16x16x4f64(af[i], bf[j], acc[i][j], 0, 0, 0);
    }
  }

#pragma unroll
  for (int i = 0; i < 4; i++) {
#pragma unroll
    for (int j = 0; j < 4; j++) {
      const size_t gcol = col0 + wc * 64 + j * 16 + fr;
#pragma unroll
      for (int rg = 0; rg < 4; rg++) {
        const size_t grow = row0 + wr * 64 + i * 16 + fq + 4 * rg;
        if (!g.lower_only || gcol <= grow) {
          double *p = g.C + grow * g.ldc + gcol;
          *p = *p - acc[i][j][rg];
        }
      }
    }
  }
}

#ifdef SINTERP_DIAG_PROF
__device__ unsigned long long g_gemm_ts[1024 * 8];
extern "C" int gsl_sinterp_hip_debug_gemm_ts(unsigned long long *out) { return (int)hipMemcpyFromSymbol(out, HIP_SYMBOL(g_gemm_ts), sizeof(g_gemm_ts)); }
extern "C" int gsl_sinterp_hip_debug_gemm_ts_clear(void)
{
  static const unsigned long long zero[1024 * 8] = {0};
  return (int)hipMemcpyToSymbol(HIP_SYMBOL(g_gemm_ts), zero, sizeof(g_gemm_ts));
}
__device__ __forceinline__ unsigned long long gemm_stamp()
{
  unsigned long long t;
  __builtin_amdgcn_sched_barrier(0);
  asm volatile("s_memtime %0\n\ts_waitcnt lgkmcnt(0)" : "=s"(t) :: "memory");
  __builtin_amdgcn_sched_barrier(0);
  return t;
}
__device__ __forceinline__ unsigned long long gemm_rstamp()
{
  unsigned long long t;
  __builtin_amdgcn_sched_barrier(0);
  asm volatile("s_memrealtime %0\n\ts_waitcnt lgkmcnt(0)" : "=s"(t) :: "memory");
  __builtin_amdgcn_sched_barrier(0);
  return t;
}
#define GEMM_TS_INIT() unsigned long long ph_[4] = {0, 0, 0, 0}, ts_ = 0; const unsigned long long t0_ = gemm_stamp(), r0_ = gemm_rstamp()
#define GEMM_TS_BEGIN() (ts_ = gemm_stamp())
#define GEMM_TS_MARK(slot) do { const unsigned long long t_ = gemm_stamp(); ph_[slot] += t_ - ts_; ts_ = t_; } while (0)
#define GEMM_TS_MARK_SEL(cond, a, b) do { const unsigned long long t_ = gemm_stamp(), d_ = t_ - ts_; const bool c_ = (cond); \
    ph_[a] += c_ ? d_ : 0ull; ph_[b] += c_ ? 0ull : d_; ts_ = t_; } while (0)
#define GEMM_TS_FINISH() do { const unsigned long long t1_ = gemm_stamp(), r1_ = gemm_rstamp(); \
    if (threadIdx.x == 0 && blockIdx.x < 1024) { unsigned long long *o_ = g_gemm_ts + blockIdx.x * 8; \
      o_[0] = t0_; o_[1] = t1_; o_[2] = ph_[0]; o_[3] = ph_[1]; o_[4] = ph_[2]; o_[5] = ph_[3]; o_[6] = r0_; o_[7] = r1_; } } while (0)
#else
#define GEMM_TS_INIT() do { } while (0)
#define GEMM_TS_BEGIN() do { } while (0)
#define GEMM_TS_MARK(slot) do { } while (0)
#define GEMM_TS_MARK_SEL(cond, a, b) do { } while (0)
#define GEMM_TS_FINISH() do { } while (0)
#endif

struct StreamK {
  unsigned steps;
  unsigned total;
  unsigned base, rem;
  unsigned dp_rounds;
  double *partial;
  unsigned *flags;
};

template <int BM, int BN>
__device__ __forceinline__ void decode_tile(const GemmArgs &g, unsigned tile, int &tm, int &tn)
{
  if (!g.lower_only) {
    tm = (int)(tile / g.tiles_n); tn = (int)(tile % g.tiles_n);
  } else {
    constexpr unsigned R = BM / BN;
    const unsigned full_rows = (unsigned)g.tiles_n / R;
    const unsigned tri = R * full_rows * (full_rows + 1) / 2;
    if (tile < tri) {
      const double t = (double)tile / (double)R;
      tm = (int)((sqrt(8.0 * t + 1.0) - 1.0) * 0.5);
      while (R * (unsigned)(tm + 1) * (unsigned)(tm + 2) / 2 <= tile) tm++;
      while (R * (unsigned)tm * (unsigned)(tm + 1) / 2 > tile) tm--;
      tn = (int)(tile - R * (unsigned)tm * (unsigned)(tm + 1) / 2);
    } else {
      const unsigned t2 = tile - tri;
      tm = (int)full_rows + (int)(t2 / g.tiles_n); tn = (int)(t2 % g.tiles_n);
    }
  }
}

template <int BM, int BN, int WM, int WN, int SS = 1, int ST = DM_STAGES, bool PIPE = false, bool BKN = false>
__global__ void __launch_bounds__((BM / WM) * (BN / WN) * 64)
gemm_minus_streamk_kernel(GemmArgs g, StreamK x)
{
  static_assert(ST == 3 || ST == 2, "ring depth");
  static_assert(!PIPE || (ST == 3 && SS == 1), "pipelined loop: three-deep ring of single steps");
  static_assert(!BKN || BN == 128, "k-row = one 1-KiB DMA instruction");
  constexpr int WCOLS = BN / WN;
  constexpr int NW = (BM / WM) * WCOLS;
  constexpr int NT = NW * 64;
  constexpr int FM = WM / 16, FN = WN / 16;
  constexpr int BPITCH = BN + 16;
  constexpr int A_TILE = BM * GT_BK, B_TILE = BKN ? GT_BK * BPITCH : BN * GT_BK;
  constexpr int A_CH = BM / 8 / NW, B_CH = (BN / 8) / NW;
  static_assert(A_CH >= 1 && B_CH >= 1 && A_CH * 8 * NW == BM && B_CH * 8 * NW == BN, "tile / wave split");
  constexpr int PER_GROUP = SS * (A_CH + B_CH);
  static_assert(PER_GROUP <= 32, "vmcnt immediate");
  constexpr size_t GK = (size_t)GT_BK * SS;
  extern __shared__ __attribute__((aligned(16))) double smem[];
  double *sA = smem;
  double *sB = smem + ST * SS * A_TILE;

  const unsigned G = gridDim.x, bid = blockIdx.x;
  const unsigned q = G / 8, r = G % 8, xcd = bid % 8;
  const unsigned gl = (xcd < r ? xcd * (q + 1) : r * (q + 1) + (xcd - r) * q) + bid / 8;
  auto start_of = [&](unsigned w) -> unsigned { return w * x.base + (w < x.rem ? w : x.rem); };
  auto start_cap = [&](unsigned w) -> unsigned { const unsigned v = start_of(w); return v < x.total ? v : x.total; };
  unsigned it = __builtin_amdgcn_readfirstlane(start_cap(gl));
  const unsigned it_end = __builtin_amdgcn_readfirstlane(start_cap(gl + 1));
  unsigned tile = __builtin_amdgcn_readfirstlane(it / x.steps);
  const unsigned dp_tiles = x.dp_rounds * G;
  unsigned round = 0;
  GEMM_TS_INIT();

  for (;;) {
    const bool dp = round < x.dp_rounds;
    if (!dp && it >= it_end) break;
    const unsigned tile_first = dp ? 0u : tile * x.steps, tile_end = tile_first + x.steps;
    const unsigned s0 = dp ? 0u : it - tile_first;
    const unsigned s1 = dp ? x.steps : (it_end < tile_end ? it_end - tile_first : x.steps);
    int tm, tn;
    {
      const unsigned tid_ = dp ? round * G + gl : dp_tiles + tile;
      decode_tile<BM, BN>(g, tid_, tm, tn);
    }
    const size_t row0 = (size_t)tm * BM, col0 = (size_t)tn * BN;
    GEMM_TS_BEGIN();

    double4_t acc[FM][FN];
    constexpr bool CPRE = FM * FN <= 8;
    double4_t cpre[CPRE ? FM : 1][CPRE ? FN : 1];
    auto load_cpre = [&]() {
      if constexpr (CPRE) {
        int tid = threadIdx.x;
        asm volatile("" : "+v"(tid));
        const int lane = tid & 63, wave = tid >> 6;
        const int wr = wave / WCOLS, wc = wave % WCOLS;
        const int fr = lane & 15, fq = lane >> 4;
#pragma unroll
        for (int i = 0; i < FM; i++)
#pragma unroll
          for (int j = 0; j < FN; j++)
#pragma unroll
            for (int rg = 0; rg < 4; rg++)
              cpre[i][j][rg] = g.C[(row0 + wr * WM + i * 16 + fq + 4 * rg) * g.ldc + col0 + wc * WN + j * 16 + fr];
      }
    };
    {
      int tid = threadIdx.x;
      asm volatile("" : "+v"(tid));
      const int lane = tid & 63, wave = tid >> 6;
      const int wr = wave / WCOLS, wc = wave % WCOLS;
      const int fr = lane & 15, fq = lane >> 4;
      const int sw = (fr >> 1) & 7;
      int koff[4];
#pragma unroll
      for (int kk = 0; kk < 4; kk++) koff[kk] = (((kk * 2 + (fq >> 1)) ^ sw) << 1) + (fq & 1);
      const int arow = (wr * WM + fr) * GT_BK, brow = BKN ? fq * BPITCH + wc * WN + fr : (wc * WN + fr) * GT_BK;

      const double *srcA[A_CH], *srcB[B_CH];
#pragma unroll
      for (int i = 0; i < A_CH; i++) {
        const int rr = (wave * A_CH + i) * 8 + (lane >> 3);
        srcA[i] = g.A + (row0 + rr) * g.lda + (((lane & 7) ^ ((rr >> 1) & 7)) << 1);
      }
#pragma unroll
      for (int i = 0; i < B_CH; i++) {
        const int rr = (wave * B_CH + i) * 8 + (lane >> 3);
        if constexpr (BKN) srcB[i] = g.B + (size_t)(wave * B_CH + i) * g.ldb + col0 + lane * 2;
        else srcB[i] = g.B + (col0 + rr) * g.ldb + (((lane & 7) ^ ((rr >> 1) & 7)) << 1);
      }
      auto issue = [&](int stage, size_t k0) {
#pragma unroll
        for (int ss = 0; ss < SS; ss++) {
#pragma unroll
          for (int i = 0; i < A_CH; i++) dma16(srcA[i] + k0 + ss * GT_BK, sA + (stage * SS + ss) * A_TILE + (wave * A_CH + i) * 128);
#pragma unroll
          for (int i = 0; i < B_CH; i++) {
            if constexpr (BKN) dma16(srcB[i] + (k0 + ss * GT_BK) * g.ldb, sB + (stage * SS + ss) * B_TILE + (wave * B_CH + i) * BPITCH);
            else dma16(srcB[i] + k0 + ss * GT_BK, sB + (stage * SS + ss) * B_TILE + (wave * B_CH + i) * 128);
          }
        }
      };

#pragma unroll
      for (int i = 0; i < FM; i++)
#pragma unroll
        for (int j = 0; j < FN; j++) acc[i][j] = (double4_t){0.0, 0.0, 0.0, 0.0};

      __syncthreads();
      if constexpr (PIPE) {
        auto wait_keep = [&](int groups) {
          static_assert(PER_GROUP == 4 || PER_GROUP == 6 || PER_GROUP == 8, "vmcnt immediate");
          if (groups >= 2) {
            if constexpr (PER_GROUP == 8) asm volatile("s_waitcnt vmcnt(16)" ::: "memory");
            else if constexpr (PER_GROUP == 6) asm volatile("s_waitcnt vmcnt(12)" ::: "memory");
            else asm volatile("s_waitcnt vmcnt(8)" ::: "memory");
          } else if (groups == 1) {
            if constexpr (PER_GROUP == 8) asm volatile("s_waitcnt vmcnt(8)" ::: "memory");
            else if constexpr (PER_GROUP == 6) asm volatile("s_waitcnt vmcnt(6)" ::: "memory");
            else asm volatile("s_waitcnt vmcnt(4)" ::: "memory");
          } else asm volatile("s_waitcnt vmcnt(0)" ::: "memory");
        };
        auto load_frag = [&](int stage, int kk, double (&af)[FM], double (&bf)[FN]) {
          const double *a_base = sA + stage * A_TILE + arow;
          const double *b_base = sB + stage * B_TILE + brow;
#pragma unroll
          for (int i = 0; i < FM; i++) af[i] = a_base[i * 16 * GT_BK + koff[kk]];
#pragma unroll
          for (int j = 0; j < FN; j++) bf[j] = BKN ? b_base[kk * 4 * BPITCH + j * 16] : b_base[j * 16 * GT_BK + koff[kk]];
        };
        auto mma = [&](const double (&af)[FM], const double (&bf)[FN]) {
#pragma unroll
          for (int i = 0; i < FM; i++)
#pragma unroll
            for (int j = 0; j < FN; j++)
              acc[i][j] = __builtin_amdgcn_mfma_f64_16x16x4f64(af[i], bf[j], acc[i][j], 0, 0, 0);
        };
        const unsigned nst = s1 - s0;
        issue(0, (size_t)s0 * GK);
        if (nst > 1) issue(1, (size_t)(s0 + 1) * GK);
        if (nst > 2) issue(2, (size_t)(s0 + 2) * GK);
        wait_keep(nst > 2 ? 2 : (int)nst - 1);
        __builtin_amdgcn_s_barrier();
        __builtin_amdgcn_sched_barrier(0);
        GEMM_TS_MARK(0);
        double af0[FM], bf0[FN], af1[FM], bf1[FN];
        load_frag(0, 0, af0, bf0);
        for (unsigned rel = 0; rel + 1 < nst; rel++) {
          const int stage = (int)(rel % 3);
          load_frag(stage, 1, af1, bf1);
          mma(af0, bf0);
          load_frag(stage, 2, af0, bf0);
          mma(af1, bf1);
          load_frag(stage, 3, af1, bf1);
          mma(af0, bf0);
          asm volatile("s_waitcnt lgkmcnt(0)" ::: "memory");
#pragma unroll
          for (int i = 0; i < FM; i++) asm volatile("" : "+v"(af1[i]));
#pragma unroll
          for (int j = 0; j < FN; j++) asm volatile("" : "+v"(bf1[j]));
          wait_keep(rel + 2 < nst ? 1 : 0);
          __builtin_amdgcn_s_barrier();
          __builtin_amdgcn_sched_barrier(0);
          if (rel + 3 < nst) issue(stage, (size_t)(s0 + rel + 3) * GK);
          load_frag((int)((rel + 1) % 3), 0, af0, bf0);
          __builtin_amdgcn_sched_barrier(0);
          mma(af1, bf1);
        }
        if (s0 == 0) load_cpre();
        {
          const int stage = (int)((nst - 1) % 3);
          load_frag(stage, 1, af1, bf1);
          mma(af0, bf0);
          load_frag(stage, 2, af0, bf0);
          mma(af1, bf1);
          load_frag(stage, 3, af1, bf1);
          mma(af0, bf0);
          mma(af1, bf1);
        }
        GEMM_TS_MARK(1);
      } else {
      issue(0, (size_t)s0 * GK);
      if (s0 + 1 < s1) issue(1, (size_t)(s0 + 1) * GK);
      for (unsigned s = s0; s < s1; s++) {
        const unsigned rel = s - s0;
        if (s + 1 < s1) {
          if constexpr (PER_GROUP == 8) asm volatile("s_waitcnt vmcnt(8)" ::: "memory");
          else if constexpr (PER_GROUP == 6) asm volatile("s_waitcnt vmcnt(6)" ::: "memory");
          else if constexpr (PER_GROUP == 4) asm volatile("s_waitcnt vmcnt(4)" ::: "memory");
          else { static_assert(PER_GROUP == 4 || PER_GROUP == 6 || PER_GROUP == 8 || PER_GROUP == 16, "vmcnt immediate"); asm volatile("s_waitcnt vmcnt(16)" ::: "memory"); }
        } else asm volatile("s_waitcnt vmcnt(0)" ::: "memory");
        __builtin_amdgcn_s_barrier();
        __builtin_amdgcn_sched_barrier(0);
        GEMM_TS_MARK_SEL(__builtin_amdgcn_readfirstlane(s) == __builtin_amdgcn_readfirstlane(s0), 0, 1);
        if (s0 == 0 && s + 1 == s1) load_cpre();
        if constexpr (ST == 3) {
          if (s + 2 < s1) issue((int)((rel + 2) % 3), (size_t)(s + 2) * GK);
        }
        const int stage = (int)(rel % ST);
#pragma unroll
        for (int ss = 0; ss < SS; ss++) {
          const double *a_base = sA + (stage * SS + ss) * A_TILE + arow;
          const double *b_base = sB + (stage * SS + ss) * B_TILE + brow;
#pragma unroll
          for (int kk = 0; kk < 4; kk++) {
            double af[FM], bf[FN];
#pragma unroll
            for (int i = 0; i < FM; i++) af[i] = a_base[i * 16 * GT_BK + koff[kk]];
#pragma unroll
            for (int j = 0; j < FN; j++) bf[j] = BKN ? b_base[kk * 4 * BPITCH + j * 16] : b_base[j * 16 * GT_BK + koff[kk]];
#pragma unroll
            for (int i = 0; i < FM; i++)
#pragma unroll
              for (int j = 0; j < FN; j++)
                acc[i][j] = __builtin_amdgcn_mfma_f64_16x16x4f64(af[i], bf[j], acc[i][j], 0, 0, 0);
          }
        }
        if constexpr (ST == 2) {
          if (s + 2 < s1) {
            __builtin_amdgcn_s_barrier();
            __builtin_amdgcn_sched_barrier(0);
            issue(stage, (size_t)(s + 2) * GK);
          }
        }
      }
      GEMM_TS_MARK(1);
      }
    }

    int tid = threadIdx.x;
    size_t row0e = row0, col0e = col0;
    asm volatile("" : "+v"(tid), "+s"(row0e), "+s"(col0e));
    const int lane = tid & 63, wave = tid >> 6;
    const int wr = wave / WCOLS, wc = wave % WCOLS;
    const int fr = lane & 15, fq = lane >> 4;
    if (s0 != 0) {
      double *pp = x.partial + (size_t)gl * (BM * BN) + tid;
#pragma unroll
      for (int i = 0; i < FM; i++) {
#pragma unroll
        for (int j = 0; j < FN; j++)
#pragma unroll
          for (int rg = 0; rg < 4; rg++)
            __hip_atomic_store(pp + ((i * FN + j) * 4 + rg) * NT, acc[i][j][rg], __ATOMIC_RELAXED, __HIP_MEMORY_SCOPE_AGENT);
        __builtin_amdgcn_sched_barrier(0);
      }
      asm volatile("s_waitcnt vmcnt(0)" ::: "memory");
      __syncthreads();
      if (tid == 0) __hip_atomic_store(x.flags + gl, 1u, __ATOMIC_RELAXED, __HIP_MEMORY_SCOPE_AGENT);
      GEMM_TS_MARK(2);
    } else {
      if (s1 < x.steps) {
        for (unsigned w = gl + 1; w < G; w++) {
          if (start_of(w) >= tile_end) break;
          if (tid == 0)
            while (__hip_atomic_load(x.flags + w, __ATOMIC_RELAXED, __HIP_MEMORY_SCOPE_AGENT) == 0u) __builtin_amdgcn_s_sleep(8);
          __syncthreads();
          const double *pp = x.partial + (size_t)w * (BM * BN) + tid;
#pragma unroll
          for (int i = 0; i < FM; i++) {
#pragma unroll
            for (int j = 0; j < FN; j++)
#pragma unroll
              for (int rg = 0; rg < 4; rg++)
                acc[i][j][rg] += __hip_atomic_load(pp + ((i * FN + j) * 4 + rg) * NT, __ATOMIC_RELAXED, __HIP_MEMORY_SCOPE_AGENT);
            __builtin_amdgcn_sched_barrier(0);
          }
          if (tid == 0) __hip_atomic_store(x.flags + w, 0u, __ATOMIC_RELAXED, __HIP_MEMORY_SCOPE_AGENT);
        }
      }
      GEMM_TS_MARK(2);
#pragma unroll
      for (int i = 0; i < FM; i++) {
#pragma unroll
        for (int j = 0; j < FN; j++) {
          const size_t gcol = col0e + wc * WN + j * 16 + fr;
#pragma unroll
          for (int rg = 0; rg < 4; rg++) {
            const size_t grow = row0e + wr * WM + i * 16 + fq + 4 * rg;
            if (!g.lower_only || gcol <= grow) {
              double *p = g.C + grow * g.ldc + gcol;
              if constexpr (CPRE) *p = cpre[i][j][rg] - acc[i][j][rg];
              else *p = *p - acc[i][j][rg];
            }
          }
        }
        __builtin_amdgcn_sched_barrier(0);
      }
#ifdef SINTERP_DIAG_PROF
      asm volatile("s_waitcnt vmcnt(0)" ::: "memory");
      GEMM_TS_MARK(3);
#endif
    }
    if (dp) round++;
    else { it = tile_first + s1; tile++; }
  }
  GEMM_TS_FINISH();
}

int sinterp_streamk_prepare(gsl_sinterp_hip_ctx *ctx)
{
  if (ctx->sk_wgs) return ST_SUCCESS;
  static const bool off = getenv("GSL_SINTERP_NO_STREAMK") && getenv("GSL_SINTERP_NO_STREAMK")[0] == '1';
  if (off) return ST_SUCCESS;
  int cus = 0;
  HIP_OK(ctx, hipDeviceGetAttribute(&cus, hipDeviceAttributeMultiprocessorCount, ctx->device));
  if (cus <= 0) return ST_SUCCESS;
  HIP_OK(ctx, hipMalloc((void **)&ctx->d_sk_partial, (size_t)cus * 256 * GT_BN * sizeof(double)));
  HIP_OK(ctx, hipMalloc((void **)&ctx->d_sk_flags, (size_t)cus * 2 * sizeof(unsigned)));
  HIP_OK(ctx, hipMemset(ctx->d_sk_flags, 0, (size_t)cus * 2 * sizeof(unsigned)));
  HIP_OK(ctx, hipDeviceSynchronize());
  ctx->sk_wgs = cus;
  return ST_SUCCESS;
}

template <int BN>
__global__ void __launch_bounds__(256)
gemm_minus_smallk_kernel(GemmArgs g)
{
  constexpr int NF = BN / 16;
  extern __shared__ __attribute__((aligned(16))) double smem[];
  const int K = (int)g.k, LD = K + 2;
  double *sA = smem;
  double *sB = smem + 128 * LD;
  const size_t row0 = (size_t)blockIdx.x * 128;
  const int tid = threadIdx.x, lane = tid & 63, wave = tid >> 6;
  const int fr = lane & 15, fq = lane >> 4;
  const int kch = K / 2;

  double4_t acc[2][NF];
#pragma unroll
  for (int i = 0; i < 2; i++)
#pragma unroll
    for (int j = 0; j < NF; j++) {
      const size_t gcol = j * 16 + fr;
#pragma unroll
      for (int rg = 0; rg < 4; rg++) {
        const size_t grow = row0 + wave * 32 + i * 16 + fq + 4 * rg;
        const size_t rcl = grow < g.m ? grow : g.m - 1;
        acc[i][j][rg] = g.C[rcl * g.ldc + gcol];
      }
    }
  for (int c = tid; c < 128 * kch; c += 256) {
    const int rr = c / kch, kc = (c % kch) * 2;
    const size_t grow = row0 + rr, rcl = grow < g.m ? grow : g.m - 1;
    const double2 v = *reinterpret_cast<const double2 *>(g.A + rcl * g.lda + kc);
    *reinterpret_cast<double2 *>(&sA[rr * LD + kc]) = make_double2(-v.x, -v.y);
  }
  for (int c = tid; c < BN * kch; c += 256) {
    const int rr = c / kch, kc = (c % kch) * 2;
    *reinterpret_cast<double2 *>(&sB[rr * LD + kc]) = *reinterpret_cast<const double2 *>(g.B + (size_t)rr * g.ldb + kc);
  }
  __syncthreads();
  const double *a_base = sA + (wave * 32 + fr) * LD + fq;
  const double *b_base = sB + fr * LD + fq;
  for (int kk = 0; kk < K; kk += 4) {
    double af[2], bf[NF];
#pragma unroll
    for (int i = 0; i < 2; i++) af[i] = a_base[i * 16 * LD + kk];
#pragma unroll
    for (int j = 0; j < NF; j++) bf[j] = b_base[j * 16 * LD + kk];
#pragma unroll
    for (int i = 0; i < 2; i++)
#pragma unroll
      for (int j = 0; j < NF; j++) acc[i][j] = __builtin_amdgcn_mfma_f64_16x16x4f64(af[i], bf[j], acc[i][j], 0, 0, 0);
  }
#pragma unroll
  for (int i = 0; i < 2; i++)
#pragma unroll
    for (int j = 0; j < NF; j++) {
      const size_t gcol = j * 16 + fr;
#pragma unroll
      for (int rg = 0; rg < 4; rg++) {
        const size_t grow = row0 + wave * 32 + i * 16 + fq + 4 * rg;
        if (grow < g.m && (!g.lower_only || gcol <= grow)) g.C[grow * g.ldc + gcol] = acc[i][j][rg];
      }
    }
}

enum { SK_256 = 0,
       SK_128 = 1,
       SK_64 = 2,
       SK_128W8 = 5,
       SK_64W8G = 6 };
static inline int sk_tile(int cfg) { return cfg == SK_128 || cfg == SK_128W8 ? 128 : cfg == SK_256 ? 256 : 64; }

template <int BM, int BN, int WM, int WN, int SS = 1, int ST = DM_STAGES, bool PIPE = false>
static int launch_sk(gsl_sinterp_hip_ctx *ctx, unsigned G, const GemmArgs &h, const StreamK &x)
{
  constexpr int NT = (BM / WM) * (BN / WN) * 64;
  const size_t lds = (size_t)ST * SS * (BM + BN) * GT_BK * sizeof(double);
  { int ast = sinterp_func_lds(ctx, (const void *)gemm_minus_streamk_kernel<BM, BN, WM, WN, SS, ST, PIPE>, (int)lds); if (ast) return ast; }
  hipLaunchKernelGGL((gemm_minus_streamk_kernel<BM, BN, WM, WN, SS, ST, PIPE>), dim3(G), dim3(NT), lds, ctx->stream, h, x);
  LAUNCH_CHECK(ctx);
  return ST_SUCCESS;
}

template <class TilesOf>
static int sk_rule(bool can256, TilesOf &tiles_of, unsigned steps, unsigned cus)
{
  GemmArgs hh;
  if (can256 && (unsigned long long)tiles_of(SK_256, hh) * steps >= 128ull * cus) return SK_256;
  if (4ull * tiles_of(SK_128, hh) <= 3ull * cus) return SK_64W8G;
  return SK_128W8;
}

static int g_gemm_last_cfg = -1;
extern "C" int gsl_sinterp_hip_debug_gemm_last_cfg(void) { return __atomic_load_n(&g_gemm_last_cfg, __ATOMIC_RELAXED); }

int sinterp_gemm_minus(gsl_sinterp_hip_ctx *ctx, size_t m, size_t n, size_t k, const double *A, size_t lda,
                       const double *B, size_t ldb, int b_is_kn, double *C, size_t ldc, int lower_only)
{
  if (m == 0 || n == 0 || k == 0) return ST_SUCCESS;
  __atomic_store_n(&g_gemm_last_cfg, -1, __ATOMIC_RELAXED);
  GemmArgs g;
  g.m = m; g.n = n; g.k = k; g.A = A; g.lda = lda; g.B = B; g.ldb = ldb; g.C = C; g.ldc = ldc;
  g.lower_only = lower_only;
  g.tiles_m = (int)((m + GT_BM - 1) / GT_BM);
  g.tiles_n = (int)((n + GT_BN - 1) / GT_BN);
  if (lower_only && g.tiles_m < g.tiles_n) g.tiles_n = g.tiles_m;
  unsigned grid = (unsigned)g.tiles_m * (unsigned)g.tiles_n;
  if (lower_only) {
    const unsigned tn_ = (unsigned)g.tiles_n;
    grid = tn_ * (tn_ + 1) / 2 + ((unsigned)g.tiles_m - tn_) * tn_;
  }
  g.n_active = grid;
  const bool full = (m % GT_BM == 0) && (n % GT_BN == 0) && (k % GT_BK == 0) && ((lda & 1) == 0) && ((ldb & 1) == 0) &&
                    ((((uintptr_t)A) & 15) == 0) && ((((uintptr_t)B) & 15) == 0);
  if (!b_is_kn && (n == 32 || n == 64) && k <= 64 && (k % 4) == 0 && k >= 4 && ((lda & 1) == 0) && ((ldb & 1) == 0) &&
      ((((uintptr_t)A) & 15) == 0) && ((((uintptr_t)B) & 15) == 0)) {
    const size_t lds = (size_t)(128 + n) * (k + 2) * sizeof(double);
    if (n == 32) {
      { int ast = sinterp_func_lds(ctx, (const void *)gemm_minus_smallk_kernel<32>, 160 * 1024); if (ast) return ast; }
      hipLaunchKernelGGL(gemm_minus_smallk_kernel<32>, dim3((unsigned)g.tiles_m), dim3(256), lds, ctx->stream, g);
    } else {
      { int ast = sinterp_func_lds(ctx, (const void *)gemm_minus_smallk_kernel<64>, 160 * 1024); if (ast) return ast; }
      hipLaunchKernelGGL(gemm_minus_smallk_kernel<64>, dim3((unsigned)g.tiles_m), dim3(256), lds, ctx->stream, g);
    }
    LAUNCH_CHECK(ctx);
    return ST_SUCCESS;
  }
  static const bool no_dma = getenv("GSL_SINTERP_NO_DMA_GEMM") && getenv("GSL_SINTERP_NO_DMA_GEMM")[0] == '1';
  if (full && !b_is_kn && k >= 4 * GT_BK && !no_dma) {
    static const bool no_w8 = getenv("GSL_SINTERP_NO_GEMM8") && getenv("GSL_SINTERP_NO_GEMM8")[0] == '1';
    if (ctx->sk_wgs > 0) {
      StreamK x;
      x.steps = (unsigned)(k / GT_BK);
      x.partial = ctx->d_sk_partial;
      x.flags = ctx->d_sk_flags;
      const unsigned cus = (unsigned)ctx->sk_wgs;
      const bool can256 = !no_w8 && (m % 256 == 0) && (!lower_only || (g.tiles_n % 2) == 0);
      auto tiles_of = [&](int c, GemmArgs &hh) -> unsigned {
        hh = g;
        if (c == SK_256) {
          hh.tiles_m = (int)(m / 256);
          if (!lower_only) return (unsigned)hh.tiles_m * (unsigned)hh.tiles_n;
          const unsigned fr_ = (unsigned)hh.tiles_n / 2;
          return 2 * fr_ * (fr_ + 1) / 2 + ((unsigned)hh.tiles_m - fr_) * (unsigned)hh.tiles_n;
        }
        const int bt = sk_tile(c);
        hh.tiles_m = (int)(m / bt); hh.tiles_n = (int)(n / bt);
        if (lower_only && hh.tiles_m < hh.tiles_n) hh.tiles_n = hh.tiles_m;
        const unsigned tm_ = (unsigned)hh.tiles_m, tn_ = (unsigned)hh.tiles_n;
        return lower_only ? tn_ * (tn_ + 1) / 2 + (tm_ - tn_) * tn_ : tm_ * tn_;
      };
      static const bool r4_rule = getenv("GSL_SINTERP_GEMM_RULE_R4") && getenv("GSL_SINTERP_GEMM_RULE_R4")[0] == '1';
      static const bool no_t64 = getenv("GSL_SINTERP_NO_GEMM64") && getenv("GSL_SINTERP_NO_GEMM64")[0] == '1';
      GemmArgs h;
      int cfg;
      bool whole = false;
      if (r4_rule) {
        cfg = SK_128;
        { GemmArgs h8; const unsigned t8 = tiles_of(SK_256, h8);
          if (can256 && (unsigned long long)t8 * x.steps >= 16ull * cus) cfg = SK_256; }
        if (cfg == SK_128 && !no_t64 && 2u * grid <= cus) cfg = SK_64;
      } else {
        cfg = sk_rule(can256, tiles_of, x.steps, cus);
        if (no_t64 && cfg == SK_64W8G) cfg = SK_128W8;
      }
      if (getenv("GSL_SINTERP_GEMM_CFG")) {
        const char *ov = getenv("GSL_SINTERP_GEMM_CFG");
        const int want_cfg = atoi(ov);
        if ((want_cfg == SK_256 && can256) || want_cfg == SK_128 || want_cfg == SK_64 || want_cfg == SK_128W8 || want_cfg == SK_64W8G) {
          cfg = want_cfg;
          whole = strchr(ov, 'w') != NULL;
        }
      }
      unsigned tiles = tiles_of(cfg, h);
      static const bool no_group = getenv("GSL_SINTERP_NO_GEMM_GROUP") && getenv("GSL_SINTERP_NO_GEMM_GROUP")[0] == '1';
      static const bool no_pipe = getenv("GSL_SINTERP_NO_GEMM_PIPE") && getenv("GSL_SINTERP_NO_GEMM_PIPE")[0] == '1';
      if (cfg == SK_64W8G && (no_group || (k % (4 * GT_BK)) != 0)) cfg = SK_64;
      const bool grouped = (cfg == SK_64 && !no_group && (k % (4 * GT_BK)) == 0) || cfg == SK_64W8G;
      if (grouped) x.steps = (unsigned)(k / (4 * GT_BK));
      static const bool no_hybrid = getenv("GSL_SINTERP_NO_HYBRID_SK") && getenv("GSL_SINTERP_NO_HYBRID_SK")[0] == '1';
      if (no_hybrid) whole = false;
      unsigned G;
      unsigned long long total64;
      if (whole) {
        G = tiles < cus ? tiles : cus;
        x.dp_rounds = tiles / G;
        total64 = (unsigned long long)(tiles - x.dp_rounds * G) * x.steps;
      } else {
        total64 = (unsigned long long)tiles * x.steps;
        unsigned long long want = total64 / (grouped ? 4 : 16);
        if (want < tiles) want = tiles;
        if (want > cus) want = cus;
        G = (unsigned)(want ? want : 1);
        x.dp_rounds = (!no_hybrid && tiles / G >= 2) ? tiles / G - 1 : 0;
        total64 = (unsigned long long)(tiles - x.dp_rounds * G) * x.steps;
      }
      if (total64 < 0x7fffffffull) {
        x.total = (unsigned)total64;
        if (whole) { x.base = x.steps; x.rem = 0; }
        else { x.base = x.total / G; x.rem = x.total % G; }
        __atomic_store_n(&g_gemm_last_cfg, 2 * cfg + (whole ? 1 : 0), __ATOMIC_RELAXED);
        switch (cfg) {
          case SK_256:
            return no_pipe ? launch_sk<256, 128, 64, 64>(ctx, G, h, x) : launch_sk<256, 128, 64, 64, 1, 3, true>(ctx, G, h, x);
          case SK_128:
            return no_pipe ? launch_sk<128, 128, 64, 64>(ctx, G, h, x) : launch_sk<128, 128, 64, 64, 1, 3, true>(ctx, G, h, x);
          case SK_128W8:
            return no_pipe ? launch_sk<128, 128, 64, 32>(ctx, G, h, x) : launch_sk<128, 128, 64, 32, 1, 3, true>(ctx, G, h, x);
          case SK_64W8G:
            return launch_sk<64, 64, 32, 16, 4, 2>(ctx, G, h, x);
          default:
            return grouped ? launch_sk<64, 64, 32, 32, 4, 2>(ctx, G, h, x) : launch_sk<64, 64, 32, 32>(ctx, G, h, x);
        }
      }
    }
    const bool w8 = !no_w8 && (m % 256 == 0) && (!lower_only || (g.tiles_n % 2) == 0) && grid >= 1024;
    if (w8) {
      GemmArgs h = g;
      h.tiles_m = (int)(m / 256);
      unsigned grid8 = (unsigned)h.tiles_m * (unsigned)h.tiles_n;
      if (lower_only) {
        const unsigned fr_ = (unsigned)h.tiles_n / 2;
        grid8 = 2 * fr_ * (fr_ + 1) / 2 + ((unsigned)h.tiles_m - fr_) * (unsigned)h.tiles_n;
      }
      const size_t lds8 = (size_t)DM_STAGES * (256 + 128) * GT_BK * sizeof(double);
      { int ast = sinterp_func_lds(ctx, (const void *)gemm_minus_dma_nt_kernel<4>, (int)lds8); if (ast) return ast; }
      hipLaunchKernelGGL(gemm_minus_dma_nt_kernel<4>, dim3(grid8), dim3(512), lds8, ctx->stream, h);
      LAUNCH_CHECK(ctx);
      return ST_SUCCESS;
    }
    const size_t lds = (size_t)DM_STAGES * (128 + 128) * GT_BK * sizeof(double);
    { int ast = sinterp_func_lds(ctx, (const void *)gemm_minus_dma_nt_kernel<2>, (int)lds); if (ast) return ast; }
    hipLaunchKernelGGL(gemm_minus_dma_nt_kernel<2>, dim3(grid), dim3(256), lds, ctx->stream, g);
    LAUNCH_CHECK(ctx);
    return ST_SUCCESS;
  }
  static const bool no_kn = getenv("GSL_SINTERP_NO_KN_STREAMK") && getenv("GSL_SINTERP_NO_KN_STREAMK")[0] == '1';
  if (b_is_kn && full && !lower_only && !no_dma && !no_kn && ctx->sk_wgs > 0 && k >= 4 * GT_BK) {
    StreamK x;
    x.steps = (unsigned)(k / GT_BK);
    x.partial = ctx->d_sk_partial; x.flags = ctx->d_sk_flags;
    GemmArgs h = g;
    unsigned tiles = grid;
    bool big = false;
    if ((m % 256) == 0) {
      const unsigned t8 = (unsigned)(m / 256) * (unsigned)g.tiles_n;
      if ((unsigned long long)t8 * x.steps >= 16ull * (unsigned)ctx->sk_wgs) { big = true; h.tiles_m = (int)(m / 256); tiles = t8; }
    }
    unsigned long long total64 = (unsigned long long)tiles * x.steps;
    unsigned long long want = total64 / 16;
    if (want < tiles) want = tiles;
    if (want > (unsigned long long)ctx->sk_wgs) want = (unsigned long long)ctx->sk_wgs;
    const unsigned G = (unsigned)(want ? want : 1);
    x.dp_rounds = (tiles / G >= 2) ? tiles / G - 1 : 0;
    total64 = (unsigned long long)(tiles - x.dp_rounds * G) * x.steps;
    if (total64 < 0x7fffffffull) {
      x.total = (unsigned)total64; x.base = x.total / G; x.rem = x.total % G;
      if (big) {
        const size_t lds = (size_t)DM_STAGES * (256 * GT_BK + GT_BK * (128 + 16)) * sizeof(double);
        { int ast = sinterp_func_lds(ctx, (const void *)gemm_minus_streamk_kernel<256, 128, 64, 64, 1, 3, true, true>, (int)lds); if (ast) return ast; }
        hipLaunchKernelGGL((gemm_minus_streamk_kernel<256, 128, 64, 64, 1, 3, true, true>), dim3(G), dim3(512), lds, ctx->stream, h, x);
      } else {
        const size_t lds = (size_t)DM_STAGES * (128 * GT_BK + GT_BK * (128 + 16)) * sizeof(double);
        { int ast = sinterp_func_lds(ctx, (const void *)gemm_minus_streamk_kernel<128, 128, 64, 64, 1, 3, true, true>, (int)lds); if (ast) return ast; }
        hipLaunchKernelGGL((gemm_minus_streamk_kernel<128, 128, 64, 64, 1, 3, true, true>), dim3(G), dim3(256), lds, ctx->stream, h, x);
      }
      LAUNCH_CHECK(ctx);
      return ST_SUCCESS;
    }
  }
  if (b_is_kn) {
    if (full) hipLaunchKernelGGL((gemm_minus_kernel<1, true>), dim3(grid), dim3(256), 0, ctx->stream, g);
    else hipLaunchKernelGGL((gemm_minus_kernel<1, false>), dim3(grid), dim3(256), 0, ctx->stream, g);
  } else {
    if (full) hipLaunchKernelGGL((gemm_minus_kernel<0, true>), dim3(grid), dim3(256), 0, ctx->stream, g);
    else hipLaunchKernelGGL((gemm_minus_kernel<0, false>), dim3(grid), dim3(256), 0, ctx->stream, g);
  }
  LAUNCH_CHECK(ctx);
  return ST_SUCCESS;
}

extern "C" int gsl_sinterp_hip_gemm_minus(gsl_sinterp_hip_ctx *ctx, size_t m, size_t n, size_t k, const double *d_a,
                                          size_t lda, const double *d_b, size_t ldb, int b_is_kn, double *d_c,
                                          size_t ldc, int lower_only)
{
  REQUIRE(ctx, ctx != NULL, ST_EFAULT);
  HIP_OK(ctx, hipSetDevice(ctx->device));
  EXCLUSIVE_SECTION(ctx);
  REQUIRE(ctx, lda >= k && ldc >= n && ldb >= (b_is_kn ? n : k), ST_EINVAL);
  REQUIRE(ctx, (m == 0 || n == 0 || k == 0) || (d_a && d_b && d_c), ST_EFAULT);
  int st = sinterp_streamk_prepare(ctx);
  if (st) return st;
  return sinterp_gemm_minus(ctx, m, n, k, d_a, lda, d_b, ldb, b_is_kn, d_c, ldc, lower_only);
}
```

Measured before the change: 31.84 M points/s.

## Fuse next diagonal-block factorization as a rider workgroup inside trailing stream-K GEMM

Adds an extra 'rider' workgroup to the stream-K trailing-update GEMM. It waits on a per-panel counter until the tiles covering the next 128-wide diagonal block are written, then factors that block in LDS, inverts it and runs the folded forward substitution. The separate chol_diag128 launch for that panel is then skipped. Those diagonal tiles are given priority and split into slices so they finish early. This is meant to take the serial diagonal factorization off the critical path between panels, at the cost of one fewer GEMM workgroup, spin polling with a timeout abort word, and more LDS per workgroup.

```diff
diff --git a/gsl-scattered-interpolation_amd/csrc/hip/chol.hip b/gsl-scattered-interpolation_amd/csrc/hip/chol.hip
--- a/gsl-scattered-interpolation_amd/csrc/hip/chol.hip
+++ b/gsl-scattered-interpolation_amd/csrc/hip/chol.hip
@@ -9,7 +9,6 @@
 #endif
 #include "chol_potrf.h"
 
-#define TRSV_MAXR 5
 
 
 __global__ void __launch_bounds__(256)
@@ -102,99 +101,12 @@
 }
 
 
-__device__ __forceinline__ void diag128_forward(const double *S, const double *Dv, double *fs, double *tt, int tid, int nrhs)
-{
-  const int lane = tid & 63, wave = tid >> 6, r = lane & 31, half = lane >> 5;
-  for (int q = wave; q < nrhs; q += 4) {
-    double *y = fs + q * PB, *t = tt + q * CB;
-#pragma unroll
-    for (int i = 0; i < 4; i++) {
-      double sum = 0.0;
-#pragma unroll
-      for (int kb = 0; kb < i; kb++) {
-        const double *Lr = S + pblk(i, kb) + r * PQ + half * 16;
-        const double *yk = y + kb * 32 + half * 16;
-#pragma unroll
-        for (int k = 0; k < 16; k += 2) {
-          const double2 l2 = *reinterpret_cast<const double2 *>(Lr + k);
-          sum = fma(l2.x, yk[k], sum);
-          sum = fma(l2.y, yk[k + 1], sum);
-        }
-      }
-      sum += __shfl_xor(sum, 32);
-      if (half == 0) t[r] = y[i * 32 + r] - sum;
-      __builtin_amdgcn_wave_barrier();
-      const double *Wr = Dv + i * PBLK + (half * 16) * PQ + r;
-      double acc = 0.0;
-#pragma unroll
-      for (int c = 0; c < 16; c++) acc = fma(Wr[c * PQ], t[half * 16 + c], acc);
-      acc += __shfl_xor(acc, 32);
-      if (half == 0) y[i * 32 + r] = acc;
-      __builtin_amdgcn_wave_barrier();
-    }
-  }
-}
-
 __global__ void __launch_bounds__(256)
 chol_diag128_kernel(double *__restrict__ A, size_t lda, size_t j0, int *__restrict__ info, double *__restrict__ diag_store,
                     double *__restrict__ Dinvg, double *__restrict__ fb, size_t ldf, int nrhs)
 {
   extern __shared__ __attribute__((aligned(16))) double sm[];
-  double *S = sm;
-  double *Dv = S + 10 * PBLK;
-  double *fs = Dv + 4 * PBLK;
-  double *tt = fs + 5 * PB;
-  const int tid = threadIdx.x;
-  double *Ab = A + j0 * lda + j0;
-  TSTAMP(0);
-
-  {
-    double v[40], fv[3];
-    const int r8 = tid >> 5, k = tid & 31;
-#pragma unroll
-    for (int t = 0; t < 40; t++) {
-      constexpr int BI[10] = {0, 1, 1, 2, 2, 2, 3, 3, 3, 3}, BJ[10] = {0, 0, 1, 0, 1, 2, 0, 1, 2, 3};
-      const int b = t >> 2, r = (t & 3) * 8 + r8;
-      v[t] = Ab[(size_t)(BI[b] * 32 + r) * lda + BJ[b] * 32 + k];
-    }
-#pragma unroll
-    for (int t = 0; t < 3; t++) { const int e = t * 256 + tid; fv[t] = e < nrhs * PB ? fb[(size_t)(e >> 7) * ldf + j0 + (e & 127)] : 0.0; }
-#pragma unroll
-    for (int t = 0; t < 40; t++) S[(t >> 2) * PBLK + ((t & 3) * 8 + r8) * PQ + k] = v[t];
-#pragma unroll
-    for (int t = 0; t < 16; t++) { const int r = (t & 3) * 8 + r8; Dv[(t >> 2) * PBLK + r * PQ + k] = r == k ? 1.0 : 0.0; }
-#pragma unroll
-    for (int t = 0; t < 3; t++) { const int e = t * 256 + tid; if (e < nrhs * PB) fs[e] = fv[t]; }
-  }
-  __syncthreads();
-  TSTAMP(1);
-
-  potrf128_lds<4>(S, Dv, tid, info, j0);
-
-  TSTAMP(18);
-  if (nrhs > 0) {
-    diag128_forward(S, Dv, fs, tt, tid, nrhs);
-    __syncthreads();
-  }
-  {
-    const int r8 = tid >> 5, k = tid & 31;
-#pragma unroll
-    for (int t = 0; t < 40; t++) {
-      constexpr int BI[10] = {0, 1, 1, 2, 2, 2, 3, 3, 3, 3}, BJ[10] = {0, 0, 1, 0, 1, 2, 0, 1, 2, 3};
-      const int b = t >> 2, r = (t & 3) * 8 + r8, bi = BI[b], bj = BJ[b];
-      const double v = S[b * PBLK + r * PQ + k];
-      if (bi != bj || k <= r) Ab[(size_t)(bi * 32 + r) * lda + bj * 32 + k] = v;
-      if (bi == bj && diag_store) diag_store[(j0 / CB + bi) * (CB * CB) + r * CB + k] = (k <= r) ? v : 0.0;
-    }
-#pragma unroll
-    for (int t = 0; t < 16; t++) {
-      const int b = t >> 2, r = (t & 3) * 8 + r8;
-      Dinvg[b * 1024 + r * 32 + k] = Dv[b * PBLK + k * PQ + r];
-    }
-#pragma unroll
-    for (int t = 0; t < 3; t++) { const int e = t * 256 + tid; if (e < nrhs * PB) fb[(size_t)(e >> 7) * ldf + j0 + (e & 127)] = fs[e]; }
-  }
-  TSTAMP(19);
+  chol_diag128_block<4>(sm, A + j0 * lda + j0, lda, j0, info, diag_store, Dinvg, fb, ldf, nrhs, threadIdx.x);
 }
 
 #define TRX 130
@@ -476,17 +388,28 @@
   return w1;
 }
 
+static int g_chol_riders_last = 0;
+extern "C" int gsl_sinterp_hip_debug_chol_riders(void) { return __atomic_load_n(&g_chol_riders_last, __ATOMIC_RELAXED); }
+
+static bool chol_rider_applicable(size_t n, const double *d_a, size_t lda)
+{
+  static const bool no_p128 = getenv("GSL_SINTERP_NO_PANEL128") && getenv("GSL_SINTERP_NO_PANEL128")[0] == '1';
+  static const bool no_rider = getenv("GSL_SINTERP_NO_DIAG_RIDER") && getenv("GSL_SINTERP_NO_DIAG_RIDER")[0] == '1';
+  return !no_p128 && !no_rider && n >= 2 * PB && n % PB == 0 && (lda & 1) == 0 && ((((uintptr_t)d_a) & 15) == 0);
+}
+
 static int chol_panel(gsl_sinterp_hip_ctx *ctx, double *A, size_t lda, size_t n, size_t j0, size_t w, int *d_info,
-                      double *d_diag, double *fb, size_t ldf, int nrhs)
+                      double *d_diag, double *fb, size_t ldf, int nrhs, unsigned *d_cnt, bool diag_done)
 {
   int st;
   static const bool no_p128 = getenv("GSL_SINTERP_NO_PANEL128") && getenv("GSL_SINTERP_NO_PANEL128")[0] == '1';
+  double *d_linv = d_diag + ((n + CB - 1) / CB) * (CB * CB);
   if (w == PB && !no_p128 && (lda & 1) == 0 && ((((uintptr_t)(A + j0 * lda + j0)) & 15) == 0)) {
-    double *d_linv = d_diag + ((n + CB - 1) / CB) * (CB * CB);
-    const size_t lds_diag = (size_t)(14 * PBLK + TRSV_MAXR * (PB + CB)) * sizeof(double);
+    const size_t lds_diag = DIAG128_LDS_BYTES;
     { int ast = sinterp_func_lds(ctx, (const void *)chol_diag128_kernel, (int)lds_diag); if (ast) return ast; }
-    hipLaunchKernelGGL(chol_diag128_kernel, dim3(1), dim3(256), lds_diag, ctx->stream, A, lda, j0, d_info,
-                       n % PB == 0 ? (double *)NULL : d_diag, d_linv, fb, ldf, nrhs);
+    if (!diag_done)
+      hipLaunchKernelGGL(chol_diag128_kernel, dim3(1), dim3(256), lds_diag, ctx->stream, A, lda, j0, d_info,
+                         n % PB == 0 ? (double *)NULL : d_diag, d_linv, fb, ldf, nrhs);
     const size_t below = n - j0 - w;
     if (below) {
       static const int force_rf = getenv("GSL_SINTERP_TRSM_RF") ? atoi(getenv("GSL_SINTERP_TRSM_RF")) : 0;
@@ -507,6 +430,7 @@
     return ST_SUCCESS;
   }
   if (w <= PB) {
+    if (diag_done) return sinterp_fail(ctx, ST_EFAILED, "cholesky: rider on a panel that is not 128 wide", hipSuccess, __FILE__, __LINE__);
     if (fb) return sinterp_fail(ctx, ST_EFAILED, "cholesky: folded forward substitution on a panel that is not 128 wide", hipSuccess, __FILE__, __LINE__);
   }
   if (w <= CB) {
@@ -517,12 +441,18 @@
     return ST_SUCCESS;
   }
   const size_t w1 = chol_split(w);
-  st = chol_panel(ctx, A, lda, n, j0, w1, d_info, d_diag, fb, ldf, nrhs);
+  st = chol_panel(ctx, A, lda, n, j0, w1, d_info, d_diag, fb, ldf, nrhs, d_cnt, diag_done);
   if (st) return st;
   const size_t r0 = j0 + w1, w2 = w - w1;
-  st = sinterp_gemm_minus(ctx, n - r0, w2, w1, A + r0 * lda + j0, lda, A + r0 * lda + j0, lda, 0, A + r0 * lda + r0, lda, 1);
+  int rode = 0;
+  sinterp_rider rd;
+  rd.info = d_info; rd.j0 = r0; rd.dinv = d_linv; rd.fb = fb; rd.ldf = ldf; rd.nrhs = nrhs;
+  rd.counter = d_cnt ? d_cnt + r0 / PB : NULL; rd.abort_word = (unsigned *)(d_info + 1);
+  st = sinterp_gemm_minus(ctx, n - r0, w2, w1, A + r0 * lda + j0, lda, A + r0 * lda + j0, lda, 0, A + r0 * lda + r0, lda, 1,
+                          d_cnt ? &rd : NULL, &rode);
   if (st) return st;
-  return chol_panel(ctx, A, lda, n, r0, w2, d_info, d_diag, fb, ldf, nrhs);
+  if (rode) ctx->chol_riders++;
+  return chol_panel(ctx, A, lda, n, r0, w2, d_info, d_diag, fb, ldf, nrhs, d_cnt, rode != 0);
 }
 
 static bool chol_fold_applicable(size_t n, const double *d_a, size_t lda, int nrhs)
@@ -533,16 +463,27 @@
 }
 
 
-__global__ void chol_zero_info_kernel(int *info) { *info = 0; }
+__global__ void __launch_bounds__(256)
+chol_zero_info_kernel(int *info, unsigned *cnt, unsigned ncnt)
+{
+  const unsigned i = blockIdx.x * 256 + threadIdx.x;
+  if (i < 2) info[i] = 0;
+  if (i < ncnt) cnt[i] = 0u;
+}
 
 static int chol_read_info(gsl_sinterp_hip_ctx *ctx, size_t n, int *h_info)
 {
   int *d_info = (int *)ctx->d_scratch + 8;
-  int info = 0;
+  int both[2] = {0, 0};
   HIP_OK(ctx, hipStreamSynchronize(ctx->stream));
-  HIP_OK(ctx, hipMemcpy(&info, d_info, sizeof(int), hipMemcpyDeviceToHost));
+  HIP_OK(ctx, hipMemcpy(both, d_info, sizeof both, hipMemcpyDeviceToHost));
   HIP_OK(ctx, hipStreamSynchronize(ctx->stream));
+  const int info = both[0];
   if (h_info) *h_info = info;
+  if (both[1]) {
+    snprintf(ctx->err, sizeof ctx->err, "cholesky_decomp1: a diagonal-block rider timed out (n = %zu)", n);
+    return ST_EFAILED;
+  }
   if (info) {
     snprintf(ctx->err, sizeof ctx->err, "cholesky_decomp1: matrix is not positive definite (pivot %d of %zu <= 0)", info, n);
     return ST_EDOM;
@@ -565,8 +506,11 @@
   const size_t nblk = (n + CB - 1) / CB;
   void *d_diag = NULL;
   const size_t n_pan = (n + PB - 1) / PB;
-  int st = sinterp_workspace(ctx, (nblk * CB * CB + (n_pan + 1) * (4 * 1024)) * sizeof(double), &d_diag);
+  const size_t diag_doubles = nblk * CB * CB + (n_pan + 1) * (4 * 1024);
+  int st = sinterp_workspace(ctx, diag_doubles * sizeof(double) + (n_pan + 4) * sizeof(unsigned), &d_diag);
   if (st) return st;
+  unsigned *d_cnt = (unsigned *)((double *)d_diag + diag_doubles);
+  const bool riders = chol_rider_applicable(n, d_a, lda);
   st = sinterp_streamk_prepare(ctx);
   if (st) return st;
   const bool fold = fb != NULL && chol_fold_applicable(n, d_a, lda, nrhs) && ldf >= n;
@@ -579,11 +523,12 @@
     hipStream_t saved;
     st = sinterp_capture_begin(ctx, &saved);
     if (st) return st;
-    hipLaunchKernelGGL(chol_zero_info_kernel, dim3(1), dim3(1), 0, ctx->stream, d_info);
+    hipLaunchKernelGGL(chol_zero_info_kernel, dim3((unsigned)((n_pan + 255) / 256)), dim3(256), 0, ctx->stream, d_info, d_cnt, (unsigned)n_pan);
+    ctx->chol_riders = 0;
     hipError_t me = hipSuccess;
     const unsigned nt = (unsigned)((n + 31) / 32);
     if (!symmetric_input) hipLaunchKernelGGL(tricpy_lower_to_upper_kernel, dim3(nt, nt), dim3(256), 0, ctx->stream, d_a, lda, n);
-    st = chol_panel(ctx, d_a, lda, n, 0, n, d_info, (double *)d_diag, fb, ldf, nrhs);
+    st = chol_panel(ctx, d_a, lda, n, 0, n, d_info, (double *)d_diag, fb, ldf, nrhs, riders ? d_cnt : NULL, false);
     {
       static const bool no_p128w = getenv("GSL_SINTERP_NO_PANEL128") && getenv("GSL_SINTERP_NO_PANEL128")[0] == '1';
       const bool all128 = !no_p128w && n % PB == 0 && (lda & 1) == 0 && ((((uintptr_t)d_a) & 15) == 0);
@@ -597,6 +542,7 @@
     if (st2) return st2;
     LAUNCH_CHECK(ctx);
   }
+  __atomic_store_n(&g_chol_riders_last, ctx->chol_riders, __ATOMIC_RELAXED);
   if (h_folded) *h_folded = fold ? 1 : 0;
   if (defer_info) return ST_SUCCESS;
   st = chol_read_info(ctx, n, h_info);
diff --git a/gsl-scattered-interpolation_amd/csrc/hip/chol_potrf.h b/gsl-scattered-interpolation_amd/csrc/hip/chol_potrf.h
--- a/gsl-scattered-interpolation_amd/csrc/hip/chol_potrf.h
+++ b/gsl-scattered-interpolation_amd/csrc/hip/chol_potrf.h
@@ -202,4 +202,108 @@
 
 }
 
+#ifndef TRSV_MAXR
+#define TRSV_MAXR 5
 #endif
+
+template <int NW>
+__device__ __forceinline__ void diag128_forward(const double *S, const double *Dv, double *fs, double *tt, int tid, int nrhs)
+{
+  const int lane = tid & 63, wave = tid >> 6, r = lane & 31, half = lane >> 5;
+  for (int q = wave; q < nrhs; q += NW) {
+    double *y = fs + q * PB, *t = tt + q * CB;
+#pragma unroll
+    for (int i = 0; i < 4; i++) {
+      double sum = 0.0;
+#pragma unroll
+      for (int kb = 0; kb < i; kb++) {
+        const double *Lr = S + pblk(i, kb) + r * PQ + half * 16;
+        const double *yk = y + kb * 32 + half * 16;
+#pragma unroll
+        for (int k = 0; k < 16; k += 2) {
+          const double2 l2 = *reinterpret_cast<const double2 *>(Lr + k);
+          sum = fma(l2.x, yk[k], sum);
+          sum = fma(l2.y, yk[k + 1], sum);
+        }
+      }
+      sum += __shfl_xor(sum, 32);
+      if (half == 0) t[r] = y[i * 32 + r] - sum;
+      __builtin_amdgcn_wave_barrier();
+      const double *Wr = Dv + i * PBLK + (half * 16) * PQ + r;
+      double acc = 0.0;
+#pragma unroll
+      for (int c = 0; c < 16; c++) acc = fma(Wr[c * PQ], t[half * 16 + c], acc);
+      acc += __shfl_xor(acc, 32);
+      if (half == 0) y[i * 32 + r] = acc;
+      __builtin_amdgcn_wave_barrier();
+    }
+  }
+}
+
+#define DIAG128_LDS_BYTES ((size_t)(14 * PBLK + TRSV_MAXR * (PB + CB)) * sizeof(double))
+
+template <int NW>
+__device__ __forceinline__ void chol_diag128_block(double *sm, double *Ab, size_t lda, size_t j0, int *info, double *diag_store,
+                                                   double *Dinvg, double *fb, size_t ldf, int nrhs, int tid)
+{
+  constexpr int NT = NW * 64;
+  constexpr int RP = NT / 32;
+  constexpr int PS = 32 / RP;
+  constexpr int FT = (TRSV_MAXR * PB + NT - 1) / NT;
+  static_assert(RP * PS == 32, "threads per workgroup");
+  double *S = sm;
+  double *Dv = S + 10 * PBLK;
+  double *fs = Dv + 4 * PBLK;
+  double *tt = fs + TRSV_MAXR * PB;
+  TSTAMP(0);
+
+  {
+    double v[10 * PS], fv[FT];
+    const int r8 = tid >> 5, k = tid & 31;
+#pragma unroll
+    for (int t = 0; t < 10 * PS; t++) {
+      constexpr int BI[10] = {0, 1, 1, 2, 2, 2, 3, 3, 3, 3}, BJ[10] = {0, 0, 1, 0, 1, 2, 0, 1, 2, 3};
+      const int b = t / PS, r = (t % PS) * RP + r8;
+      v[t] = Ab[(size_t)(BI[b] * 32 + r) * lda + BJ[b] * 32 + k];
+    }
+#pragma unroll
+    for (int t = 0; t < FT; t++) { const int e = t * NT + tid; fv[t] = e < nrhs * PB ? fb[(size_t)(e >> 7) * ldf + j0 + (e & 127)] : 0.0; }
+#pragma unroll
+    for (int t = 0; t < 10 * PS; t++) S[(t / PS) * PBLK + ((t % PS) * RP + r8) * PQ + k] = v[t];
+#pragma unroll
+    for (int t = 0; t < 4 * PS; t++) { const int r = (t % PS) * RP + r8; Dv[(t / PS) * PBLK + r * PQ + k] = r == k ? 1.0 : 0.0; }
+#pragma unroll
+    for (int t = 0; t < FT; t++) { const int e = t * NT + tid; if (e < nrhs * PB) fs[e] = fv[t]; }
+  }
+  __syncthreads();
+  TSTAMP(1);
+
+  potrf128_lds<NW>(S, Dv, tid, info, j0);
+
+  TSTAMP(18);
+  if (nrhs > 0) {
+    diag128_forward<NW>(S, Dv, fs, tt, tid, nrhs);
+    __syncthreads();
+  }
+  {
+    const int r8 = tid >> 5, k = tid & 31;
+#pragma unroll
+    for (int t = 0; t < 10 * PS; t++) {
+      constexpr int BI[10] = {0, 1, 1, 2, 2, 2, 3, 3, 3, 3}, BJ[10] = {0, 0, 1, 0, 1, 2, 0, 1, 2, 3};
+      const int b = t / PS, r = (t % PS) * RP + r8, bi = BI[b], bj = BJ[b];
+      const double v = S[b * PBLK + r * PQ + k];
+      if (bi != bj || k <= r) Ab[(size_t)(bi * 32 + r) * lda + bj * 32 + k] = v;
+      if (bi == bj && diag_store) diag_store[(j0 / CB + bi) * (CB * CB) + r * CB + k] = (k <= r) ? v : 0.0;
+    }
+#pragma unroll
+    for (int t = 0; t < 4 * PS; t++) {
+      const int b = t / PS, r = (t % PS) * RP + r8;
+      Dinvg[b * 1024 + r * 32 + k] = Dv[b * PBLK + k * PQ + r];
+    }
+#pragma unroll
+    for (int t = 0; t < FT; t++) { const int e = t * NT + tid; if (e < nrhs * PB) fb[(size_t)(e >> 7) * ldf + j0 + (e & 127)] = fs[e]; }
+  }
+  TSTAMP(19);
+}
+
+#endif
diff --git a/gsl-scattered-interpolation_amd/csrc/hip/common.h b/gsl-scattered-interpolation_amd/csrc/hip/common.h
--- a/gsl-scattered-interpolation_amd/csrc/hip/common.h
+++ b/gsl-scattered-interpolation_amd/csrc/hip/common.h
@@ -40,6 +40,7 @@
   double *d_sk_partial;
   unsigned *d_sk_flags;
   int sk_wgs;
+  int chol_riders;
   unsigned *d_tf;
   size_t tf_count;
   unsigned long long *d_xq;
@@ -110,8 +111,17 @@
 
 int sinterp_workspace(gsl_sinterp_hip_ctx *ctx, size_t bytes, void **out);
 
+struct sinterp_rider {
+  int *info;
+  size_t j0;
+  double *dinv;
+  double *fb; size_t ldf; int nrhs;
+  unsigned *counter;
+  unsigned *abort_word;
+};
 int sinterp_gemm_minus(gsl_sinterp_hip_ctx *ctx, size_t m, size_t n, size_t k, const double *A, size_t lda,
-                       const double *B, size_t ldb, int b_is_kn, double *C, size_t ldc, int lower_only);
+                       const double *B, size_t ldb, int b_is_kn, double *C, size_t ldc, int lower_only,
+                       const sinterp_rider *rider = NULL, int *attached = NULL);
 
 int sinterp_streamk_prepare(gsl_sinterp_hip_ctx *ctx);
 
diff --git a/gsl-scattered-interpolation_amd/csrc/hip/gemm.hip b/gsl-scattered-interpolation_amd/csrc/hip/gemm.hip
--- a/gsl-scattered-interpolation_amd/csrc/hip/gemm.hip
+++ b/gsl-scattered-interpolation_amd/csrc/hip/gemm.hip
@@ -1,8 +1,7 @@
 #include "common.h"
 #include <stdlib.h>
 #include <string.h>
-
-typedef double double4_t __attribute__((ext_vector_type(4)));
+#include "chol_potrf.h"
 
 #define GT_BM 128
 #define GT_BN 128
@@ -332,7 +331,38 @@
   unsigned dp_rounds;
   double *partial;
   unsigned *flags;
+  unsigned pri_tiles, pri_sl, pri_nsl;
+  unsigned pri_base;
 };
+
+struct RiderArgs {
+  int *info; size_t j0; double *dinv; double *fb; size_t ldf; int nrhs;
+  unsigned *counter, *abort_word;
+  unsigned need;
+};
+#define SK_PRI_SLOTS 32
+#define RIDER_MAX_POLLS (1u << 22)
+
+template <int NW>
+__device__ __forceinline__ void gemm_rider(const GemmArgs &g, const RiderArgs &rd, double *smem)
+{
+  const int tid = threadIdx.x;
+  unsigned *okw = reinterpret_cast<unsigned *>(smem + DIAG128_LDS_BYTES / sizeof(double));
+  if (tid == 0) {
+    unsigned ok = 0;
+    for (unsigned spins = 0; spins < RIDER_MAX_POLLS; spins++) {
+      if (__hip_atomic_load(rd.counter, __ATOMIC_RELAXED, __HIP_MEMORY_SCOPE_AGENT) >= rd.need) { ok = 1; break; }
+      __builtin_amdgcn_s_sleep(32);
+    }
+    if (ok) __builtin_amdgcn_fence(__ATOMIC_ACQUIRE, "agent");
+    else __hip_atomic_store(rd.abort_word, 1u, __ATOMIC_RELAXED, __HIP_MEMORY_SCOPE_AGENT);
+    *okw = ok;
+  }
+  asm volatile("s_waitcnt vmcnt(0) lgkmcnt(0)" ::: "memory");
+  __syncthreads();
+  if (*okw == 0) return;
+  chol_diag128_block<NW>(smem, g.C, g.ldc, rd.j0, rd.info, (double *)nullptr, rd.dinv, rd.fb, rd.ldf, rd.nrhs, tid);
+}
 
 template <int BM, int BN>
 __device__ __forceinline__ void decode_tile(const GemmArgs &g, unsigned tile, int &tm, int &tn)
@@ -356,9 +386,9 @@
   }
 }
 
-template <int BM, int BN, int WM, int WN, int SS = 1, int ST = DM_STAGES, bool PIPE = false, bool BKN = false>
+template <int BM, int BN, int WM, int WN, int SS = 1, int ST = DM_STAGES, bool PIPE = false, bool BKN = false, bool RIDER = false>
 __global__ void __launch_bounds__((BM / WM) * (BN / WN) * 64)
-gemm_minus_streamk_kernel(GemmArgs g, StreamK x)
+gemm_minus_streamk_kernel(GemmArgs g, StreamK x, RiderArgs rd)
 {
   static_assert(ST == 3 || ST == 2, "ring depth");
   static_assert(!PIPE || (ST == 3 && SS == 1), "pipelined loop: three-deep ring of single steps");
@@ -378,29 +408,45 @@
   double *sA = smem;
   double *sB = smem + ST * SS * A_TILE;
 
-  const unsigned G = gridDim.x, bid = blockIdx.x;
+  static_assert(!RIDER || (!BKN && NW == 8 && BM <= 128), "rider: N.T updates on 8 waves");
+  if constexpr (RIDER) {
+    if (blockIdx.x == gridDim.x - 1) { gemm_rider<NW>(g, rd, smem); return; }
+  }
+  const unsigned G = gridDim.x - (RIDER ? 1u : 0u), bid = blockIdx.x;
   const unsigned q = G / 8, r = G % 8, xcd = bid % 8;
   const unsigned gl = (xcd < r ? xcd * (q + 1) : r * (q + 1) + (xcd - r) * q) + bid / 8;
-  auto start_of = [&](unsigned w) -> unsigned { return w * x.base + (w < x.rem ? w : x.rem); };
+  constexpr bool PRI = RIDER;
+  constexpr unsigned PRI_SLOT_SCALE = (256 * GT_BN) / (BM * BN);
+  const unsigned pri_wgs = PRI ? x.pri_tiles * x.pri_nsl : 0u;
+  auto start_of = [&](unsigned w) -> unsigned {
+    const unsigned v = w * x.base + (w < x.rem ? w : x.rem);
+    if constexpr (PRI) return v - (w < pri_wgs ? w : pri_wgs) * x.pri_sl;
+    return v;
+  };
   auto start_cap = [&](unsigned w) -> unsigned { const unsigned v = start_of(w); return v < x.total ? v : x.total; };
   unsigned it = __builtin_amdgcn_readfirstlane(start_cap(gl));
   const unsigned it_end = __builtin_amdgcn_readfirstlane(start_cap(gl + 1));
   unsigned tile = __builtin_amdgcn_readfirstlane(it / x.steps);
   const unsigned dp_tiles = x.dp_rounds * G;
   unsigned round = 0;
+  bool pri_pending = PRI && gl < pri_wgs;
   GEMM_TS_INIT();
 
   for (;;) {
     const bool dp = round < x.dp_rounds;
-    if (!dp && it >= it_end) break;
-    const unsigned tile_first = dp ? 0u : tile * x.steps, tile_end = tile_first + x.steps;
-    const unsigned s0 = dp ? 0u : it - tile_first;
-    const unsigned s1 = dp ? x.steps : (it_end < tile_end ? it_end - tile_first : x.steps);
+    const bool pr = PRI && pri_pending;
+    if (!dp && !pr && it >= it_end) break;
+    const unsigned tile_first = (dp || pr) ? 0u : tile * x.steps, tile_end = tile_first + x.steps;
+    unsigned s0 = dp ? 0u : it - tile_first;
+    unsigned s1 = dp ? x.steps : (it_end < tile_end ? it_end - tile_first : x.steps);
+    unsigned gtile = dp ? round * G + gl : dp_tiles + tile;
+    if constexpr (PRI) {
+      if (pr) { s0 = (gl % x.pri_nsl) * x.pri_sl; s1 = s0 + x.pri_sl; gtile = gl / x.pri_nsl; }
+      else if (!dp) gtile += x.pri_tiles;
+    }
+    const bool hand = RIDER && gtile < rd.need;
     int tm, tn;
-    {
-      const unsigned tid_ = dp ? round * G + gl : dp_tiles + tile;
-      decode_tile<BM, BN>(g, tid_, tm, tn);
-    }
+    decode_tile<BM, BN>(g, gtile, tm, tn);
     const size_t row0 = (size_t)tm * BM, col0 = (size_t)tn * BN;
     GEMM_TS_BEGIN();
 
@@ -593,7 +639,7 @@
     const int wr = wave / WCOLS, wc = wave % WCOLS;
     const int fr = lane & 15, fq = lane >> 4;
     if (s0 != 0) {
-      double *pp = x.partial + (size_t)gl * (BM * BN) + tid;
+      double *pp = x.partial + (size_t)(gl + (pr ? x.pri_base * PRI_SLOT_SCALE : 0u)) * (BM * BN) + tid;
 #pragma unroll
       for (int i = 0; i < FM; i++) {
 #pragma unroll
@@ -605,16 +651,18 @@
       }
       asm volatile("s_waitcnt vmcnt(0)" ::: "memory");
       __syncthreads();
-      if (tid == 0) __hip_atomic_store(x.flags + gl, 1u, __ATOMIC_RELAXED, __HIP_MEMORY_SCOPE_AGENT);
+      if (tid == 0) __hip_atomic_store(x.flags + gl + (pr ? x.pri_base : 0u), 1u, __ATOMIC_RELAXED, __HIP_MEMORY_SCOPE_AGENT);
       GEMM_TS_MARK(2);
     } else {
       if (s1 < x.steps) {
+        unsigned *const fl = x.flags + (pr ? x.pri_base : 0u);
+        const double *const pbase = x.partial + (size_t)(pr ? x.pri_base * PRI_SLOT_SCALE : 0u) * (BM * BN);
         for (unsigned w = gl + 1; w < G; w++) {
-          if (start_of(w) >= tile_end) break;
+          if (pr ? w >= gl + x.pri_nsl : start_of(w) >= tile_end) break;
           if (tid == 0)
-            while (__hip_atomic_load(x.flags + w, __ATOMIC_RELAXED, __HIP_MEMORY_SCOPE_AGENT) == 0u) __builtin_amdgcn_s_sleep(8);
+            while (__hip_atomic_load(fl + w, __ATOMIC_RELAXED, __HIP_MEMORY_SCOPE_AGENT) == 0u) __builtin_amdgcn_s_sleep(8);
           __syncthreads();
-          const double *pp = x.partial + (size_t)w * (BM * BN) + tid;
+          const double *pp = pbase + (size_t)w * (BM * BN) + tid;
 #pragma unroll
           for (int i = 0; i < FM; i++) {
 #pragma unroll
@@ -624,7 +672,7 @@
                 acc[i][j][rg] += __hip_atomic_load(pp + ((i * FN + j) * 4 + rg) * NT, __ATOMIC_RELAXED, __HIP_MEMORY_SCOPE_AGENT);
             __builtin_amdgcn_sched_barrier(0);
           }
-          if (tid == 0) __hip_atomic_store(x.flags + w, 0u, __ATOMIC_RELAXED, __HIP_MEMORY_SCOPE_AGENT);
+          if (tid == 0) __hip_atomic_store(fl + w, 0u, __ATOMIC_RELAXED, __HIP_MEMORY_SCOPE_AGENT);
         }
       }
       GEMM_TS_MARK(2);
@@ -638,12 +686,22 @@
             const size_t grow = row0e + wr * WM + i * 16 + fq + 4 * rg;
             if (!g.lower_only || gcol <= grow) {
               double *p = g.C + grow * g.ldc + gcol;
-              if constexpr (CPRE) *p = cpre[i][j][rg] - acc[i][j][rg];
-              else *p = *p - acc[i][j][rg];
+              double v;
+              if constexpr (CPRE) v = cpre[i][j][rg] - acc[i][j][rg];
+              else v = *p - acc[i][j][rg];
+              if (hand) __hip_atomic_store(p, v, __ATOMIC_RELAXED, __HIP_MEMORY_SCOPE_AGENT);
+              else *p = v;
             }
           }
         }
         __builtin_amdgcn_sched_barrier(0);
+      }
+      if constexpr (RIDER) {
+        if (hand) {
+          asm volatile("s_waitcnt vmcnt(0)" ::: "memory");
+          __syncthreads();
+          if (tid == 0) __hip_atomic_fetch_add(rd.counter, 1u, __ATOMIC_RELAXED, __HIP_MEMORY_SCOPE_AGENT);
+        }
       }
 #ifdef SINTERP_DIAG_PROF
       asm volatile("s_waitcnt vmcnt(0)" ::: "memory");
@@ -651,6 +709,7 @@
 #endif
     }
     if (dp) round++;
+    else if (pr) pri_pending = false;
     else { it = tile_first + s1; tile++; }
   }
   GEMM_TS_FINISH();
@@ -664,7 +723,7 @@
   int cus = 0;
   HIP_OK(ctx, hipDeviceGetAttribute(&cus, hipDeviceAttributeMultiprocessorCount, ctx->device));
   if (cus <= 0) return ST_SUCCESS;
-  HIP_OK(ctx, hipMalloc((void **)&ctx->d_sk_partial, (size_t)cus * 256 * GT_BN * sizeof(double)));
+  HIP_OK(ctx, hipMalloc((void **)&ctx->d_sk_partial, (size_t)(cus + SK_PRI_SLOTS) * 256 * GT_BN * sizeof(double)));
   HIP_OK(ctx, hipMalloc((void **)&ctx->d_sk_flags, (size_t)cus * 2 * sizeof(unsigned)));
   HIP_OK(ctx, hipMemset(ctx->d_sk_flags, 0, (size_t)cus * 2 * sizeof(unsigned)));
   HIP_OK(ctx, hipDeviceSynchronize());
@@ -743,13 +802,14 @@
        SK_64W8G = 6 };
 static inline int sk_tile(int cfg) { return cfg == SK_128 || cfg == SK_128W8 ? 128 : cfg == SK_256 ? 256 : 64; }
 
-template <int BM, int BN, int WM, int WN, int SS = 1, int ST = DM_STAGES, bool PIPE = false>
-static int launch_sk(gsl_sinterp_hip_ctx *ctx, unsigned G, const GemmArgs &h, const StreamK &x)
+template <int BM, int BN, int WM, int WN, int SS = 1, int ST = DM_STAGES, bool PIPE = false, bool RIDER = false>
+static int launch_sk(gsl_sinterp_hip_ctx *ctx, unsigned G, const GemmArgs &h, const StreamK &x, const RiderArgs &rd = RiderArgs())
 {
   constexpr int NT = (BM / WM) * (BN / WN) * 64;
-  const size_t lds = (size_t)ST * SS * (BM + BN) * GT_BK * sizeof(double);
-  { int ast = sinterp_func_lds(ctx, (const void *)gemm_minus_streamk_kernel<BM, BN, WM, WN, SS, ST, PIPE>, (int)lds); if (ast) return ast; }
-  hipLaunchKernelGGL((gemm_minus_streamk_kernel<BM, BN, WM, WN, SS, ST, PIPE>), dim3(G), dim3(NT), lds, ctx->stream, h, x);
+  size_t lds = (size_t)ST * SS * (BM + BN) * GT_BK * sizeof(double);
+  if (RIDER && lds < DIAG128_LDS_BYTES + 16) lds = DIAG128_LDS_BYTES + 16;
+  { int ast = sinterp_func_lds(ctx, (const void *)gemm_minus_streamk_kernel<BM, BN, WM, WN, SS, ST, PIPE, false, RIDER>, (int)lds); if (ast) return ast; }
+  hipLaunchKernelGGL((gemm_minus_streamk_kernel<BM, BN, WM, WN, SS, ST, PIPE, false, RIDER>), dim3(G + (RIDER ? 1u : 0u)), dim3(NT), lds, ctx->stream, h, x, rd);
   LAUNCH_CHECK(ctx);
   return ST_SUCCESS;
 }
@@ -767,8 +827,10 @@
 extern "C" int gsl_sinterp_hip_debug_gemm_last_cfg(void) { return __atomic_load_n(&g_gemm_last_cfg, __ATOMIC_RELAXED); }
 
 int sinterp_gemm_minus(gsl_sinterp_hip_ctx *ctx, size_t m, size_t n, size_t k, const double *A, size_t lda,
-                       const double *B, size_t ldb, int b_is_kn, double *C, size_t ldc, int lower_only)
-{
+                       const double *B, size_t ldb, int b_is_kn, double *C, size_t ldc, int lower_only,
+                       const sinterp_rider *rider, int *attached)
+{
+  if (attached) *attached = 0;
   if (m == 0 || n == 0 || k == 0) return ST_SUCCESS;
   __atomic_store_n(&g_gemm_last_cfg, -1, __ATOMIC_RELAXED);
   GemmArgs g;
@@ -852,6 +914,12 @@
       if (grouped) x.steps = (unsigned)(k / (4 * GT_BK));
       static const bool no_hybrid = getenv("GSL_SINTERP_NO_HYBRID_SK") && getenv("GSL_SINTERP_NO_HYBRID_SK")[0] == '1';
       if (no_hybrid) whole = false;
+      const bool ride = rider && attached && lower_only && m >= 128 && n >= 128 && cus >= 2 && !whole &&
+                        ((cfg == SK_128W8 && !no_pipe) || cfg == SK_64W8G) &&
+                        ((((uintptr_t)C) & 15) == 0) && (ldc & 1) == 0;
+      const unsigned cus_g = ride ? cus - 1 : cus;
+      x.pri_tiles = 0; x.pri_sl = 0; x.pri_nsl = 1;
+      x.pri_base = cus;
       unsigned G;
       unsigned long long total64;
       if (whole) {
@@ -862,7 +930,7 @@
         total64 = (unsigned long long)tiles * x.steps;
         unsigned long long want = total64 / (grouped ? 4 : 16);
         if (want < tiles) want = tiles;
-        if (want > cus) want = cus;
+        if (want > cus_g) want = cus_g;
         G = (unsigned)(want ? want : 1);
         x.dp_rounds = (!no_hybrid && tiles / G >= 2) ? tiles / G - 1 : 0;
         total64 = (unsigned long long)(tiles - x.dp_rounds * G) * x.steps;
@@ -871,6 +939,27 @@
         x.total = (unsigned)total64;
         if (whole) { x.base = x.steps; x.rem = 0; }
         else { x.base = x.total / G; x.rem = x.total % G; }
+        RiderArgs rd = RiderArgs();
+        if (ride) {
+          rd.info = rider->info; rd.j0 = rider->j0; rd.dinv = rider->dinv; rd.fb = rider->fb; rd.ldf = rider->ldf;
+          rd.nrhs = rider->fb ? rider->nrhs : 0; rd.counter = rider->counter; rd.abort_word = rider->abort_word;
+          rd.need = cfg == SK_64W8G ? 3u : 1u;
+          if (x.dp_rounds == 0) {
+            static const int s_env = getenv("GSL_SINTERP_RIDER_SLICES") ? atoi(getenv("GSL_SINTERP_RIDER_SLICES")) : 0;
+            unsigned S = s_env > 0 ? (unsigned)s_env : 4u;
+            if (S > x.steps) S = x.steps;
+            while (S > 1 && (x.steps % S) != 0) S--;
+            while (S > 1 && (rd.need * S > G || rd.need * S > SK_PRI_SLOTS || 2 * (x.steps / S) > x.base || rd.need >= tiles)) {
+              S--;
+              while (S > 1 && (x.steps % S) != 0) S--;
+            }
+            if (S > 1) {
+              x.pri_tiles = rd.need; x.pri_nsl = S; x.pri_sl = x.steps / S;
+              x.total -= rd.need * x.steps;
+            }
+          }
+          *attached = 1;
+        }
         __atomic_store_n(&g_gemm_last_cfg, 2 * cfg + (whole ? 1 : 0), __ATOMIC_RELAXED);
         switch (cfg) {
           case SK_256:
@@ -878,8 +967,10 @@
           case SK_128:
             return no_pipe ? launch_sk<128, 128, 64, 64>(ctx, G, h, x) : launch_sk<128, 128, 64, 64, 1, 3, true>(ctx, G, h, x);
           case SK_128W8:
+            if (ride) return launch_sk<128, 128, 64, 32, 1, 3, true, true>(ctx, G, h, x, rd);
             return no_pipe ? launch_sk<128, 128, 64, 32>(ctx, G, h, x) : launch_sk<128, 128, 64, 32, 1, 3, true>(ctx, G, h, x);
           case SK_64W8G:
+            if (ride) return launch_sk<64, 64, 32, 16, 4, 2, false, true>(ctx, G, h, x, rd);
             return launch_sk<64, 64, 32, 16, 4, 2>(ctx, G, h, x);
           default:
             return grouped ? launch_sk<64, 64, 32, 32, 4, 2>(ctx, G, h, x) : launch_sk<64, 64, 32, 32>(ctx, G, h, x);
@@ -912,6 +1003,7 @@
     StreamK x;
     x.steps = (unsigned)(k / GT_BK);
     x.partial = ctx->d_sk_partial; x.flags = ctx->d_sk_flags;
+    x.pri_tiles = 0; x.pri_sl = 0; x.pri_nsl = 1; x.pri_base = 0;
     GemmArgs h = g;
     unsigned tiles = grid;
     bool big = false;
@@ -931,11 +1023,11 @@
       if (big) {
         const size_t lds = (size_t)DM_STAGES * (256 * GT_BK + GT_BK * (128 + 16)) * sizeof(double);
         { int ast = sinterp_func_lds(ctx, (const void *)gemm_minus_streamk_kernel<256, 128, 64, 64, 1, 3, true, true>, (int)lds); if (ast) return ast; }
-        hipLaunchKernelGGL((gemm_minus_streamk_kernel<256, 128, 64, 64, 1, 3, true, true>), dim3(G), dim3(512), lds, ctx->stream, h, x);
+        hipLaunchKernelGGL((gemm_minus_streamk_kernel<256, 128, 64, 64, 1, 3, true, true>), dim3(G), dim3(512), lds, ctx->stream, h, x, RiderArgs());
       } else {
         const size_t lds = (size_t)DM_STAGES * (128 * GT_BK + GT_BK * (128 + 16)) * sizeof(double);
         { int ast = sinterp_func_lds(ctx, (const void *)gemm_minus_streamk_kernel<128, 128, 64, 64, 1, 3, true, true>, (int)lds); if (ast) return ast; }
-        hipLaunchKernelGGL((gemm_minus_streamk_kernel<128, 128, 64, 64, 1, 3, true, true>), dim3(G), dim3(256), lds, ctx->stream, h, x);
+        hipLaunchKernelGGL((gemm_minus_streamk_kernel<128, 128, 64, 64, 1, 3, true, true>), dim3(G), dim3(256), lds, ctx->stream, h, x, RiderArgs());
       }
       LAUNCH_CHECK(ctx);
       return ST_SUCCESS;
```

Result: faster. 32.82 M points/s, median of 6 (+3.1%).
